# refresh-bio/colord

Hardware: AMD Instinct MI355X
Metric: input Gbases/s + archive size vs ref, ONT 50 Gb at 1/2/4/8 MI355X (higher is better)
Workload: dtype u64

## Files before the change

colord_amd/_native.py:

```python
from __future__ import annotations
import ctypes as C
import os

os.environ.setdefault("GPU_MAX_HW_QUEUES", "32")
_HERE = os.path.dirname(os.path.abspath(__file__))
LIB_PATH = os.environ.get("COLORD_HIP_LIBRARY") or os.path.join(_HERE, "libcolord_hip.so")

CL_OK, CL_E_INVALID, CL_E_HIP, CL_E_CAPACITY, CL_E_NOMEM, CL_E_UNSUPPORTED, CL_E_MISMATCH = 0, -1, -2, -3, -4, -5, -6


class ColordHipError(RuntimeError):
    def __init__(self, status, msg):
        super().__init__(f"colord_hip error {status}: {msg}")
        self.status = status


class QualParams(C.Structure):
    _fields_ = [("mode", C.c_int32), ("source", C.c_int32), ("level", C.c_int32), ("n_fwd", C.c_uint32), ("fwd", C.c_uint32 * 8),
                ("n_rev", C.c_uint32), ("rev", C.c_uint32 * 8)]


class KmerStats(C.Structure):
    _fields_ = [("n_reads", C.c_uint64), ("tot_kmers", C.c_uint64), ("n_unique", C.c_uint64),
                ("n_unique_counted", C.c_uint64), ("total_count_filtered", C.c_uint64)]


class Digest(C.Structure):
    _fields_ = [("reads", C.c_uint64), ("symbols", C.c_uint64), ("sum", C.c_uint64)]

    def triple(self):
        return self.reads, self.symbols, self.sum


class Report(C.Structure):
    _fields_ = [("reads", C.c_uint64), ("bases", C.c_uint64), ("base_count", C.c_uint64 * 5), ("len_min", C.c_uint64), ("len_max", C.c_uint64),
                ("len_hist", C.c_uint64 * 33), ("len_bases", C.c_uint64 * 33), ("has_qual", C.c_uint64), ("q_reads", C.c_uint64), ("q_symbols", C.c_uint64),
                ("mean_q_hist", C.c_uint64 * 96), ("q_joint", (C.c_uint64 * 96) * 96)]

    def as_dict(self):
        import numpy as np
        out = {}
        for name, t in self._fields_:
            v = getattr(self, name)
            out[name] = int(v) if t is C.c_uint64 else np.ctypeslib.as_array(v).copy()
        return out


_P = C.c_void_p
class CompressParams(C.Structure):
    _fields_ = [("k", C.c_uint32), ("f", C.c_uint32), ("ci", C.c_uint32), ("cs", C.c_uint32), ("c", C.c_uint32),
                ("anchor_len", C.c_uint32), ("min_part_alt", C.c_uint32), ("max_rec", C.c_uint32), ("min_anchors", C.c_uint32),
                ("level", C.c_int32), ("source", C.c_int32), ("sparse", C.c_int32),
                ("sparse_g", C.c_double), ("sparse_exponent", C.c_double),
                ("cost_mult", C.c_double), ("frac_always", C.c_double), ("frac_min", C.c_double), ("max_matches_mult", C.c_double)]


class CompressInfo(C.Structure):
    _fields_ = [(n, C.c_uint64) for n in ("n_reads", "n_bases", "tot_kmers", "n_kept_kmers", "n_refs", "n_anchors", "tuple_bytes", "dna_bytes", "qual_bytes")] + \
               [("sparse_range", C.c_uint32), ("pad", C.c_uint32)]


_EXCH_GATHER_HOST = C.CFUNCTYPE(C.c_int32, C.c_void_p, C.POINTER(C.c_uint64), C.c_uint32, C.POINTER(C.c_uint64))
_EXCH_A2AV = C.CFUNCTYPE(C.c_int32, C.c_void_p, C.c_void_p, C.POINTER(C.c_uint64), C.c_void_p, C.POINTER(C.c_uint64))
_EXCH_GATHERV = C.CFUNCTYPE(C.c_int32, C.c_void_p, C.c_void_p, C.c_uint64, C.c_void_p, C.POINTER(C.c_uint64))


class Exchange(C.Structure):
    _fields_ = [("user", C.c_void_p), ("rank", C.c_uint32), ("world", C.c_uint32),
                ("all_gather_host", _EXCH_GATHER_HOST), ("all_to_all_v", _EXCH_A2AV), ("all_gather_v", _EXCH_GATHERV)]


_SIG = {
    "cl_ctx_create": (C.c_int32, [C.c_int, C.POINTER(_P)]),
    "cl_ctx_destroy": (None, [_P]),
    "cl_last_error": (C.c_char_p, [_P]),
    "cl_ctx_stream": (_P, [_P]),
    "cl_ctx_last_kernel_ms": (C.c_int32, [_P, C.c_char_p, C.POINTER(C.c_double), C.POINTER(C.c_uint32)]),
    "cl_ctx_set_timing": (None, [_P, C.c_int]),
    "cl_ctx_set_verify": (None, [_P, C.c_int]),
    "cl_ctx_verified": (C.c_int32, [_P, C.POINTER(C.c_uint64), C.POINTER(C.c_uint64)]),
    "cl_ctx_gap_paths": (C.c_int32, [_P, C.POINTER(C.c_uint64), C.c_uint32]),
    "cl_ctx_set_verify_streams": (None, [_P, C.c_int]),
    "cl_ctx_verified_streams": (C.c_int32, [_P, C.POINTER(C.c_uint64), C.POINTER(C.c_uint64), C.POINTER(C.c_uint64)]),
    "cl_compressor_verified_streams": (C.c_int32, [_P, C.POINTER(C.c_uint64), C.POINTER(C.c_uint64), C.POINTER(C.c_uint64)]),
    "cl_ctx_set_digest": (None, [_P, C.c_int]),
    "cl_ctx_digest": (C.c_int32, [_P, C.POINTER(Digest), C.POINTER(Digest)]),
    "cl_compressor_digest": (C.c_int32, [_P, C.POINTER(Digest), C.POINTER(Digest)]),
    "cl_ctx_set_digest_values": (None, [_P, C.c_int]),
    "cl_ctx_digest_values": (C.c_int32, [_P, C.POINTER(Digest)]),
    "cl_compressor_digest_values": (C.c_int32, [_P, C.POINTER(Digest)]),
    "cl_digest_qual_values": (C.c_int32, [_P, C.POINTER(QualParams), _P, _P, _P, C.c_uint64, C.POINTER(Digest)]),
    "cl_qual_values": (C.c_int32, [_P, C.POINTER(QualParams), _P, _P, _P, _P, C.c_uint64]),
    "cl_qual_values_host": (C.c_int32, [C.POINTER(QualParams), _P, _P, C.c_uint64, _P]),
    "cl_digest_qual_values_host": (C.c_int32, [_P, _P, C.c_uint64, C.c_uint64, C.POINTER(Digest)]),
    "cl_report_clear": (None, [C.POINTER(Report)]),
    "cl_report_add": (None, [C.POINTER(Report), C.POINTER(Report)]),
    "cl_report_bases": (C.c_int32, [_P, _P, C.POINTER(Report)]),
    "cl_report_quals": (C.c_int32, [_P, C.POINTER(QualParams), _P, _P, _P, C.c_uint64, C.c_uint32, C.POINTER(Report)]),
    "cl_report_bases_host": (C.c_int32, [_P, _P, C.c_uint64, C.POINTER(Report)]),
    "cl_report_quals_host": (C.c_int32, [C.POINTER(QualParams), _P, _P, C.c_uint64, C.POINTER(Report)]),
    "cl_report_values_host": (C.c_int32, [_P, _P, C.c_uint64, C.POINTER(Report)]),
    "cl_ctx_set_report": (None, [_P, C.c_int]),
    "cl_ctx_report": (C.c_int32, [_P, C.POINTER(Report)]),
    "cl_compressor_report": (C.c_int32, [_P, C.POINTER(Report)]),
    "cl_digest_bases": (C.c_int32, [_P, _P, C.c_uint64, C.POINTER(Digest)]),
    "cl_digest_quals": (C.c_int32, [_P, C.POINTER(QualParams), _P, _P, _P, C.c_uint64, C.POINTER(Digest)]),
    "cl_digest_bases_host": (C.c_int32, [_P, _P, C.c_uint64, C.c_uint64, C.POINTER(Digest)]),
    "cl_digest_bytes_host": (C.c_int32, [C.c_uint32, _P, _P, C.c_uint64, C.c_uint64, C.POINTER(Digest)]),
    "cl_qual_decoder_set_digest": (C.c_int32, [_P, C.c_int, C.c_uint64]),
    "cl_qual_decoder_digest": (C.c_int32, [_P, C.POINTER(Digest)]),
    "cl_es_expand": (C.c_int32, [_P, _P, _P, _P, _P, C.c_uint32, _P, C.c_uint64, _P, C.POINTER(C.c_uint64)]),
    "cl_es_verify": (C.c_int32, [_P, _P, _P, _P, _P, _P, C.POINTER(C.c_uint64), C.POINTER(C.c_uint32)]),
    "cl_compressor_verified": (C.c_int32, [_P, C.POINTER(C.c_uint64), C.POINTER(C.c_uint64)]),
    "cl_ctx_kernel_times": (C.c_int32, [_P, C.c_char_p, C.c_uint64, C.POINTER(C.c_uint64)]),
    "cl_reads_pack": (C.c_int32, [_P, _P, _P, C.c_uint32, C.c_int, C.POINTER(_P)]),
    "cl_reads_free": (None, [_P]),
    "cl_reads_count": (C.c_uint32, [_P]),
    "cl_reads_total_bases": (C.c_uint64, [_P]),
    "cl_reads_total_words": (C.c_uint64, [_P]),
    "cl_reads_packed": (_P, [_P]),
    "cl_reads_invalid": (_P, [_P]),
    "cl_reads_word_offsets": (_P, [_P]),
    "cl_reads_lengths": (_P, [_P]),
    "cl_reads_has_n": (_P, [_P]),
    "cl_reads_compact": (C.c_int32, [_P, _P, C.c_uint32, _P, C.c_uint64, C.POINTER(C.c_uint64)]),
    "cl_kmer_scan": (C.c_int32, [_P, _P, C.c_uint32, C.c_uint32, _P, C.c_uint64, C.POINTER(C.c_uint64)]),
    "cl_kmer_count_filter": (C.c_int32, [_P, _P, C.c_uint64, C.c_uint32, C.c_uint32, C.c_uint32, C.POINTER(_P), C.POINTER(KmerStats)]),
    "cl_kmer_set_create": (C.c_int32, [_P, _P, _P, C.c_uint64, C.c_uint32, C.POINTER(_P)]),
    "cl_kmer_set_free": (None, [_P]),
    "cl_kmer_set_size": (C.c_uint64, [_P]),
    "cl_kmer_set_keys": (_P, [_P]),
    "cl_kmer_set_counts": (_P, [_P]),
    "cl_kmer_set_check": (C.c_int32, [_P, _P, _P, C.c_uint64, _P]),
    "cl_accepted_kmers": (C.c_int32, [_P, _P, _P, C.c_uint32, C.c_uint32, C.POINTER(_P)]),
    "cl_kmer_lists_free": (None, [_P]),
    "cl_kmer_lists_reads": (C.c_uint32, [_P]),
    "cl_kmer_lists_total": (C.c_uint64, [_P]),
    "cl_kmer_lists_offsets": (_P, [_P]),
    "cl_kmer_lists_kmers": (_P, [_P]),
    "cl_kmer_lists_ids": (_P, [_P]),
    "cl_kmer_lists_pos": (_P, [_P]),
    "cl_ref_accept": (C.c_int32, [C.c_uint32, C.c_uint32, C.c_uint32, C.c_double, _P]),
    "cl_index_build": (C.c_int32, [_P, _P, _P, _P, C.c_uint32, C.c_uint32, C.POINTER(_P)]),
    "cl_index_entries_of": (C.c_int32, [_P, _P, _P, C.c_uint32, _P, _P, C.c_uint64, C.POINTER(C.c_uint64), _P, C.POINTER(C.c_uint32)]),
    "cl_index_build_pairs": (C.c_int32, [_P, _P, _P, _P, C.c_uint64, _P, C.c_uint32, C.c_uint32, C.c_uint32, C.c_uint32, C.POINTER(_P)]),
    "cl_index_free": (None, [_P]),
    "cl_index_n_refs": (C.c_uint32, [_P]),
    "cl_index_entries": (C.c_uint64, [_P]),
    "cl_index_ref_rank": (_P, [_P]),
    "cl_candidates": (C.c_int32, [_P, _P, _P, C.c_uint32, _P, _P, _P]),
    "cl_candidates_common": (C.c_int32, [_P, _P, _P, C.c_uint32, _P, _P, _P, _P, C.c_uint64, C.POINTER(C.c_uint64)]),
    "cl_qual_coder_create": (C.c_int32, [_P, C.POINTER(QualParams), C.POINTER(_P)]),
    "cl_qual_coder_ctx": (_P, [_P]),
    "cl_qual_coder_free": (None, [_P]),
    "cl_qual_coder_set_domain_symbols": (C.c_int32, [_P, C.c_uint64]),
    "cl_qual_coder_domains": (C.c_int32, [_P, _P, C.c_uint64, C.POINTER(C.c_uint64)]),
    "cl_qual_coder_model": (C.c_int32, [_P, C.c_uint32, C.c_uint64, _P, C.c_uint32, C.POINTER(C.c_uint32)]),
    "cl_qual_coder_groups": (C.c_int32, [_P, C.POINTER(C.c_uint64)]),
    "cl_compressor_set_qual_domain_symbols": (C.c_int32, [_P, C.c_uint64]),
    "cl_compressor_qual_domains": (C.c_int32, [_P, _P, C.c_uint64, C.POINTER(C.c_uint64)]),
    "cl_qual_decode_domains": (C.c_int32, [_P, C.POINTER(QualParams), _P, _P, _P, C.c_uint64, _P, _P, C.c_uint32, _P, C.c_uint32, C.c_uint32, _P, _P, C.c_uint64, _P, C.c_uint64]),
    "cl_qual_encode": (C.c_int32, [_P, _P, _P, _P, _P, _P, _P, C.c_uint32, _P, C.c_uint64, _P, C.POINTER(C.c_uint64)]),
    "cl_anchor_candidates": (C.c_int32, [_P, _P, _P, _P, _P, C.c_uint32, C.c_uint32, C.c_double, C.c_double, C.c_double, C.c_uint32, C.POINTER(_P)]),
    "cl_anchor_candidates_hifi": (C.c_int32, [_P, _P, _P, _P, _P, C.c_uint32, C.c_uint32, C.c_double, C.c_double, C.c_double, C.c_uint32, C.c_uint32, C.c_uint32, _P, _P, C.POINTER(_P)]),
    "cl_anchors_free": (None, [_P]),
    "cl_anchors_total": (C.c_uint64, [_P]),
    "cl_anchors_n_cands": (_P, [_P]),
    "cl_anchors_cands": (_P, [_P]),
    "cl_anchors_cand_offsets": (_P, [_P]),
    "cl_anchors_data": (_P, [_P]),
    "cl_encode_plain": (C.c_int32, [_P, _P, _P, C.c_uint64, _P, _P, C.POINTER(C.c_uint64)]),
    "cl_reads_select": (C.c_int32, [_P, _P, _P, C.POINTER(_P)]),
    "cl_reads_from_arena": (C.c_int32, [_P, _P, _P, _P, C.c_uint32, C.POINTER(_P)]),
    "cl_estimator_logs": (C.c_int32, [_P, _P, _P, C.c_uint64, _P]),
    "cl_es_flags": (C.c_int32, [_P, _P, _P, _P, _P, _P]),
    "cl_id_coder_create": (C.c_int32, [C.c_int32, C.POINTER(_P)]),
    "cl_id_coder_free": (None, [_P]),
    "cl_id_coder_error": (C.c_char_p, [_P]),
    "cl_id_encode_part": (C.c_int32, [_P, _P, _P, _P, C.c_uint32, _P, C.c_uint64, C.POINTER(C.c_uint64)]),
    "cl_compress_shard": (C.c_int32, [_P, C.POINTER(CompressParams), _P, _P, _P, _P, C.c_uint32, _P, C.c_uint32, _P, _P, _P, C.c_uint64, _P, _P, C.c_uint64, _P,
                                      C.POINTER(CompressInfo)]),
    "cl_candidates_at": (C.c_int32, [_P, _P, _P, _P, C.c_uint32, _P, _P, _P]),
    "cl_compressor_create": (C.c_int32, [_P, _P, C.POINTER(CompressParams), C.POINTER(QualParams), C.POINTER(Exchange), C.c_uint64, C.POINTER(_P)]),
    "cl_compressor_free": (None, [_P]),
    "cl_compressor_count_add": (C.c_int32, [_P, _P]),
    "cl_compressor_count_finish": (C.c_int32, [_P, C.POINTER(KmerStats)]),
    "cl_compressor_refs_add": (C.c_int32, [_P, _P]),
    "cl_compressor_refs_finish": (C.c_int32, [_P]),
    "cl_compressor_encode": (C.c_int32, [_P, _P, _P, _P, _P, C.c_uint32, _P, C.c_uint32, _P, C.c_uint64, _P, _P, C.c_uint64, _P, C.POINTER(CompressInfo)]),
    "cl_compressor_genome_add": (C.c_int32, [_P, _P]),
    "cl_compressor_pseudo_reads": (C.c_int32, [_P, _P]),
    "cl_genome_encode": (C.c_int32, [_P, _P, C.c_uint32, _P, C.c_uint64, C.POINTER(C.c_uint64)]),
    "cl_genome_decode": (C.c_int32, [_P, C.c_uint64, C.c_uint32, _P, C.c_uint64, _P, C.POINTER(C.c_uint64)]),
    "cl_genome_md5": (C.c_int32, [_P, _P, C.c_uint32, _P]),
    "cl_compressor_prepare": (C.c_int32, [_P, _P, _P, C.c_uint32]),
    "cl_compressor_prepare_parts": (C.c_int32, [_P, _P, _P, C.c_uint32, _P, C.c_uint32, _P, _P]),
    "cl_compressor_info": (C.c_int32, [_P, C.POINTER(KmerStats), C.POINTER(C.c_uint64), C.POINTER(C.c_uint64), C.POINTER(C.c_uint64), C.POINTER(C.c_uint32), C.POINTER(C.c_uint32)]),
    "cl_dna_decoder_create": (C.c_int32, [C.c_uint32, C.c_int32, C.c_uint32, C.c_uint32, C.c_int32, C.c_uint32, C.c_double, C.POINTER(_P)]),
    "cl_dna_decoder_free": (None, [_P]),
    "cl_dna_decoder_error": (C.c_char_p, [_P]),
    "cl_dna_decoder_add_ref": (C.c_int32, [_P, _P, C.c_uint32]),
    "cl_dna_decoder_new_domain": (C.c_int32, [_P]),
    "cl_dna_decode_part": (C.c_int32, [_P, _P, C.c_uint64, C.c_uint32, _P, C.c_uint64, _P, C.POINTER(C.c_uint64)]),
    "cl_qual_decoder_create": (C.c_int32, [C.POINTER(QualParams), C.POINTER(_P)]),
    "cl_qual_decoder_free": (None, [_P]),
    "cl_qual_decoder_new_domain": (C.c_int32, [_P]),
    "cl_qual_decode_part": (C.c_int32, [_P, _P, C.c_uint64, _P, _P, C.c_uint32, _P]),
    "cl_id_decoder_create": (C.c_int32, [C.c_int32, C.POINTER(_P)]),
    "cl_id_decoder_free": (None, [_P]),
    "cl_id_decode_part": (C.c_int32, [_P, _P, C.c_uint64, C.c_uint32, _P, C.c_uint64, _P, _P, C.POINTER(C.c_uint64)]),
    "cl_encode_reads": (C.c_int32, [_P, _P, _P, _P, C.c_uint32, C.c_uint32, C.c_uint32, C.c_uint32, C.c_double, _P, C.c_uint32, _P, C.c_uint64, _P, _P, C.POINTER(C.c_uint64)]),
    "cl_dna_coder_create": (C.c_int32, [_P, C.c_uint32, C.c_int32, C.c_uint32, C.POINTER(_P)]),
    "cl_dna_coder_free": (None, [_P]),
    "cl_dna_coder_model": (C.c_int32, [_P, C.c_uint32, C.c_uint64, _P]),
    "cl_dna_encode": (C.c_int32, [_P, _P, _P, _P, _P, _P, C.c_uint32, _P, C.c_uint32, _P, C.c_uint64, _P, C.POINTER(C.c_uint64)]),
    "cl_sort_u64": (C.c_int32, [_P, _P, C.c_uint64, C.c_uint32, C.c_uint32]),
    "cl_sort_u64_u32": (C.c_int32, [_P, _P, _P, C.c_uint64, C.c_uint32, C.c_uint32]),
    "cl_sort_u32": (C.c_int32, [_P, _P, C.c_uint64, C.c_uint32, C.c_uint32]),
    "cl_sort_u32_u32": (C.c_int32, [_P, _P, _P, C.c_uint64, C.c_uint32, C.c_uint32]),
    "cl_sort_swap_u32_u32": (C.c_int32, [_P, _P, _P, C.c_uint64, C.c_uint32, C.c_uint32, _P, _P]),
    "cl_sort_swap_u64_u32": (C.c_int32, [_P, _P, _P, C.c_uint64, C.c_uint32, C.c_uint32, _P, _P]),
    "cl_scan_u32": (C.c_int32, [_P, _P, C.c_uint64, C.POINTER(C.c_uint64)]),
    "cl_scan_u32_u64": (C.c_int32, [_P, _P, _P, C.c_uint64, C.POINTER(C.c_uint64)]),
    "cl_run_starts_u32": (C.c_int32, [_P, _P, C.c_uint64, C.c_uint32, _P, C.c_uint64, C.POINTER(C.c_uint64)]),
    "cl_run_starts_u64": (C.c_int32, [_P, _P, C.c_uint64, C.c_uint32, _P, C.c_uint64, C.POINTER(C.c_uint64)]),
}

_lib = None


def load():
    global _lib
    if _lib is None:
        if not os.path.exists(LIB_PATH):
            raise ColordHipError(CL_E_HIP, f"{LIB_PATH} is missing: run `make -C colord_amd/csrc` "
                                 "(or __graft_entry__.build()); there is no CPU fallback")
        lib = C.CDLL(LIB_PATH)
        for name, (res, args) in _SIG.items():
            fn = getattr(lib, name)
            fn.restype, fn.argtypes = res, args
        _lib = lib
    return _lib


def exported_names():
    return sorted(_SIG)
```

colord_amd/csrc/anchors.hip:

```cpp
#include "common.hpp"
#include "objects.hpp"
#include <algorithm>

struct cl_anchors {
	cl_ctx* ctx = nullptr;
	uint32_t n_reads = 0, c = 0;
	uint64_t n_anchors = 0;
	DevBuf<uint32_t> n_cands;
	DevBuf<uint32_t> cand;
	DevBuf<uint64_t> cand_off;
	DevBuf<uint32_t> anchors;
};

namespace {

struct Arena { const uint64_t* packed; const uint64_t* word_off; const uint32_t* lens; };

__device__ inline uint64_t mmer_at(const Arena& A, uint64_t wb, uint32_t p, uint32_t m)
{
	const uint64_t* w = A.packed + wb + (p >> 5);
	const uint32_t j = p & 31;
	const uint64_t hi = w[0], lo = w[1];
	const uint32_t s = 128 - 2 * (j + m);
	const uint64_t v = (s >= 64) ? (hi >> (s - 64)) : ((hi << (64 - s)) | (lo >> s));
// ... 686 lines not shown
		if (ku != 2) { sel_task[n] = (trc + ku) | 0x80000000u; sel_tot[n] = k_tot[trc + ku]; sel_n[n] = k_n[trc + ku]; ++n; continue; }
		int pick = -1;
		if (arc && afw) pick = t_tot[tfw] > t_tot[trc] ? 1 : 0;
		else if (arc) pick = 0;
		else if (afw) pick = 1;
		if (pick >= 0) { sel_task[n] = trc + (uint32_t)pick; sel_tot[n] = t_tot[trc + pick]; sel_n[n] = t_nanch[trc + pick]; ++n; }
	}
	for (uint32_t i = 1; i < n; ++i)
	{
		uint32_t xt = sel_task[i], xv = sel_tot[i], xn = sel_n[i]; uint32_t j = i;
		while (j > 0 && xv > sel_tot[j - 1]) { sel_task[j] = sel_task[j - 1]; sel_tot[j] = sel_tot[j - 1]; sel_n[j] = sel_n[j - 1]; --j; }
		sel_task[j] = xt; sel_tot[j] = xv; sel_n[j] = xn;
	}
	o_ncand[r] = n;
	for (uint32_t i = 0; i < c; ++i)
	{
		const uint64_t s = (uint64_t)r * c + i;
		if (i < n)
		{
			const uint32_t t = sel_task[i] & 0x7fffffffu, slot = (t / 2) % c;
			o_cand[4 * s] = cand_refs[(uint64_t)r * c + slot]; o_cand[4 * s + 1] = (t & 1) == 0 ? 1u : 0u;
			o_cand[4 * s + 2] = sel_tot[i]; o_cand[4 * s + 3] = sel_n[i];
			o_task[(uint64_t)rl * c + i] = sel_task[i]; o_count[(uint64_t)rl * c + i] = sel_n[i];
		}
		else { o_cand[4 * s] = ~0u; o_cand[4 * s + 1] = 0; o_cand[4 * s + 2] = 0; o_cand[4 * s + 3] = 0; o_task[(uint64_t)rl * c + i] = ~0u; o_count[(uint64_t)rl * c + i] = 0; }
	}
}
__global__ void k_copy_fix(const uint32_t* __restrict__ o_task, const uint64_t* __restrict__ slot_off, uint64_t n_slots,
                           const uint64_t* __restrict__ pair_off, const uint32_t* __restrict__ anch, uint64_t dst_base, uint32_t* __restrict__ out,
                           TaskCfg cfg, const uint32_t* __restrict__ kanch, const uint64_t* __restrict__ common_off, uint64_t common_base)
{
	const uint64_t s = (uint64_t)blockIdx.x * blockDim.x + threadIdx.x;
	if (s >= n_slots) return;
	const uint32_t tm = o_task[s];
	if (tm == ~0u) return;
	const uint32_t t = tm & 0x7fffffffu;
	const uint32_t n = (uint32_t)(slot_off[s + 1] - slot_off[s]);
	const uint32_t* src = anch + 3 * pair_off[t];
	if (tm & 0x80000000u)
	{
		const uint64_t gs = (uint64_t)cfg.r0 * cfg.c + t / 2;
		const uint64_t o = common_off[gs] - common_base; const uint32_t nk = (uint32_t)(common_off[gs + 1] - common_off[gs]);
		src = kanch + 6 * o + (uint64_t)(t & 1) * 3 * nk;
	}
	uint32_t* dst = out + 3 * (dst_base + slot_off[s]);
	for (uint32_t i = 0; i < 3 * n; ++i) dst[i] = src[i];
	for (uint32_t i = 0; i + 1 < n; ++i)
	{
		const uint32_t end = dst[3 * i + 2] + dst[3 * i];
		if (dst[3 * (i + 1) + 2] < end) { const uint32_t d = end - dst[3 * (i + 1) + 2]; dst[3 * (i + 1) + 2] += d; dst[3 * (i + 1)] -= d; dst[3 * (i + 1) + 1] += d; }
	}
	for (uint32_t i = 0; i + 1 < n; ++i)
	{
		const uint32_t end = dst[3 * i + 1] + dst[3 * i];
		if (dst[3 * (i + 1) + 1] < end) { const uint32_t d = end - dst[3 * (i + 1) + 1]; dst[3 * (i + 1) + 1] += d; dst[3 * (i + 1)] -= d; dst[3 * (i + 1) + 2] += d; }
	}
}
__global__ void k_add_u64(uint64_t* v, uint64_t n, uint64_t c) { uint64_t i = (uint64_t)blockIdx.x * blockDim.x + threadIdx.x; if (i < n) v[i] += c; }
}

extern "C" cl_status cl_anchor_candidates_hifi(cl_ctx* ctx, const cl_reads* reads, const cl_reads* refs, const uint32_t* d_cand_refs, const uint32_t* d_cand_n,
                                               uint32_t c, uint32_t anchor_len, double frac_always, double frac_min, double max_matches_mult,
                                               uint32_t min_anchors, uint32_t kmer_len, uint32_t modulo, const uint64_t* d_common_off, const uint64_t* d_common, cl_anchors** out);
extern "C" cl_status cl_anchor_candidates(cl_ctx* ctx, const cl_reads* reads, const cl_reads* refs, const uint32_t* d_cand_refs, const uint32_t* d_cand_n,
                                          uint32_t c, uint32_t anchor_len, double frac_always, double frac_min, double max_matches_mult,
                                          uint32_t min_anchors, cl_anchors** out)
{
	return cl_anchor_candidates_hifi(ctx, reads, refs, d_cand_refs, d_cand_n, c, anchor_len, frac_always, frac_min, max_matches_mult, min_anchors, 0, 0, nullptr, nullptr, out);
}
extern "C" cl_status cl_anchor_candidates_hifi(cl_ctx* ctx, const cl_reads* reads, const cl_reads* refs, const uint32_t* d_cand_refs, const uint32_t* d_cand_n,
                                               uint32_t c, uint32_t anchor_len, double frac_always, double frac_min, double max_matches_mult,
                                               uint32_t min_anchors, uint32_t kmer_len, uint32_t modulo, const uint64_t* d_common_off, const uint64_t* d_common, cl_anchors** out)
{
	if (!ctx || !reads || !refs || !d_cand_refs || !d_cand_n || !out) return cl_fail(ctx, CL_E_INVALID, "cl_anchor_candidates: null argument");
	const bool hifi = d_common_off != nullptr;
	if (hifi && (kmer_len < 2 || kmer_len > 28 || modulo == 0)) return cl_fail(ctx, CL_E_INVALID, "cl_anchor_candidates_hifi: 2 <= kmer_len <= 28, modulo >= 1");
	if (c == 0 || c > 16 || anchor_len < 2 || anchor_len > 28) return cl_fail(ctx, CL_E_INVALID, "cl_anchor_candidates: 1 <= c <= 16, 2 <= anchor_len <= 28");
	HIP_TRY(ctx, hipSetDevice(ctx->device));
	const uint32_t nr = reads->n_reads, m = anchor_len;
	cl_anchors* X = new cl_anchors(); X->ctx = ctx; X->n_reads = nr; X->c = c;
	std::unique_ptr<cl_anchors> guard(X);
	DEV_ALLOC(ctx, X->n_cands, nr); DEV_ALLOC(ctx, X->cand, (uint64_t)nr * c * 4); DEV_ALLOC(ctx, X->cand_off, (uint64_t)nr * c + 1);
	Arena A{ reads->packed.p, reads->word_off.p, reads->lens.p }, R{ refs->packed.p, refs->word_off.p, refs->lens.p };
	std::vector<uint32_t> h_len(nr);
	if (nr) HIP_TRY(ctx, hipMemcpy(h_len.data(), reads->lens.p, (uint64_t)nr * 4, hipMemcpyDeviceToHost));
	auto bits_for = [](uint64_t v) -> uint32_t { uint32_t b = 1; while ((1ull << b) <= v) ++b; return b; };
	uint32_t max_ref_len = 0;
	if (refs->n_reads)
	{
		std::vector<uint32_t> rl(refs->n_reads);
		HIP_TRY(ctx, hipMemcpy(rl.data(), refs->lens.p, (uint64_t)refs->n_reads * 4, hipMemcpyDeviceToHost));
		for (uint32_t l : rl) max_ref_len = std::max(max_ref_len, l);
	}
	const uint32_t pr_bits = bits_for(max_ref_len);
	const uint64_t BATCH_BASES = 1ull << 28;
	std::vector<DevBuf<uint32_t>> chunks; std::vector<uint64_t> chunk_n;
	uint64_t total_anchors = 0;
	double pairs_per_base = 0.5;
	struct TableBatch {
		uint32_t r0 = 0, r1 = 0, pe = 1; uint64_t acc = 0, nsum = 0;
		DevBuf<uint32_t> n_distinct, next, err; DevBuf<uint64_t> toff, noff; DevBuf<EncSlot> slots; DevBuf<uint2> bins;
		std::vector<uint2> h_work; DevBuf<uint2> work;
		struct SideSync { hipStream_t s = nullptr; ~SideSync() { if (s) (void)hipStreamSynchronize(s); } } sync;
	};
	HIP_TRY(ctx, cl_side_stream(ctx, ctx->side));
	constexpr uint32_t LDS_N_A = 12288, LDS_N_B = 24576, LDS_NT = 1024;
	uint32_t lds_max_n = 0;
	if (const char* e = getenv("COLORD_HIP_ANCHORS_LDS")) lds_max_n = atoi(e) <= 0 ? 0u : (uint32_t)atoi(e) <= LDS_N_A ? LDS_N_A : LDS_N_B;
	const uint32_t match_seg = getenv("COLORD_HIP_MATCH_SEG") ? (uint32_t)std::max(0, atoi(getenv("COLORD_HIP_MATCH_SEG"))) : 16384u;
	const uint32_t lds_dbg = getenv("COLORD_HIP_LDS_DBG") ? (uint32_t)atoi(getenv("COLORD_HIP_LDS_DBG")) : 0u;
	auto prepare = [&](uint32_t r0, std::unique_ptr<TableBatch>& out) -> cl_status {
		out = std::make_unique<TableBatch>();
		TableBatch& B = *out;
		uint32_t r1 = r0; uint64_t acc = 0;
		uint32_t mx = 0;
		while (r1 < nr && (r1 == r0 || acc + h_len[r1] <= BATCH_BASES))
		{
			const uint32_t pe = bits_for(std::max(mx, h_len[r1]));
			if (r1 > r0 && pe + pr_bits + bits_for((r1 - r0 + 1) * 2 * c) > 64) break;
			mx = std::max(mx, h_len[r1]); acc += h_len[r1]; ++r1;
		}
		B.r0 = r0; B.r1 = r1; B.acc = acc; B.pe = bits_for(mx);
		for (uint32_t r = r0; r < r1; ++r)
			for (uint32_t sg = 0, ns = match_segments(h_len[r] >= m ? h_len[r] - m + 1 : 0, match_seg); sg < ns; ++sg) B.h_work.push_back(make_uint2(r - r0, sg));
		if (B.pe + pr_bits + bits_for((r1 - r0) * 2 * c) > 64) return cl_fail(ctx, CL_E_UNSUPPORTED, "cl_anchor_candidates: a read and its candidates are too long for 64-bit match keys");
		const uint32_t nb = r1 - r0;
		const uint32_t table_x4 = 8;
		LaunchOn on(ctx, ctx->side);
		B.sync.s = ctx->side;
		DevBuf<uint32_t> tsize, nsize, err; DEV_ALLOC(ctx, tsize, nb); DEV_ALLOC(ctx, nsize, nb); DEV_ALLOC(ctx, err, 1); DEV_ALLOC(ctx, B.n_distinct, nb);
		HIP_TRY(ctx, hipMemsetAsync(err.p, 0, 4, ctx->side));
		LAUNCH(ctx, k_table_sizes, grid_for(nb, 256), 256, (const uint32_t*)reads->lens.p, (const uint8_t*)reads->has_n.p, d_cand_n, r0, r1, m, table_x4, lds_max_n, tsize.p, nsize.p, err.p);
		DEV_ALLOC(ctx, B.toff, (uint64_t)nb + 1); DEV_ALLOC(ctx, B.noff, (uint64_t)nb + 1);
		uint64_t tsum = 0;
		CL_TRY(dev_exclusive_scan_u64(ctx, tsize.p, B.toff.p, nb, &tsum));
		CL_TRY(dev_exclusive_scan_u64(ctx, nsize.p, B.noff.p, nb, &B.nsum));
		uint32_t herr = 0; HIP_TRY(ctx, hipMemcpyAsync(&herr, err.p, 4, hipMemcpyDeviceToHost, ctx->side)); HIP_TRY(ctx, hipStreamSynchronize(ctx->side));
		DEV_ALLOC(ctx, B.slots, tsum); DEV_ALLOC(ctx, B.next, B.nsum); DEV_ALLOC(ctx, B.bins, B.nsum); DEV_ALLOC(ctx, B.err, 1);
		DEV_ALLOC(ctx, B.work, B.h_work.size() + 1);
		if (!B.h_work.empty()) HIP_TRY(ctx, hipMemcpyAsync(B.work.p, B.h_work.data(), B.h_work.size() * sizeof(uint2), hipMemcpyHostToDevice, ctx->side));
		HIP_TRY(ctx, hipMemsetAsync(B.n_distinct.p, 0, (uint64_t)nb * 4, ctx->side));
		HIP_TRY(ctx, hipMemsetAsync(B.err.p, 0, 4, ctx->side));
		EncTable T{ B.slots.p, B.toff.p, B.next.p, B.noff.p };
		LAUNCHB(ctx, B.nsum * (0.25 + 16.0) , k_table_insert, nb, INS_T, A, r0, r1, m, T, B.n_distinct.p, B.bins.p, B.err.p);
		HIP_TRY(ctx, hipGetLastError());
		return CL_OK;
	};
	std::unique_ptr<TableBatch> cur, nxt;
	if (nr) CL_TRY(prepare(0, cur));
	while (cur)
	{
		const uint32_t r0 = cur->r0, r1 = cur->r1; const uint64_t acc = cur->acc;
		const uint32_t nb = r1 - r0, n_tasks = nb * 2 * c;
		TaskCfg cfg{ r0, r1, c, m, cur->pe, pr_bits, frac_always, frac_min, max_matches_mult };
		HIP_TRY(ctx, hipStreamSynchronize(ctx->stream));
		HIP_TRY(ctx, hipStreamSynchronize(ctx->side));
		cur->sync.s = nullptr;
		{ uint32_t herr = 0; HIP_TRY(ctx, hipMemcpy(&herr, cur->err.p, 4, hipMemcpyDeviceToHost)); if (herr) return cl_fail(ctx, CL_E_UNSUPPORTED, "cl_anchor_candidates: a region of an m-mer table overflowed"); }
		DevBuf<uint32_t>& n_distinct = cur->n_distinct;
		EncTable T{ cur->slots.p, cur->toff.p, cur->next.p, cur->noff.p };
		DevBuf<uint32_t> pair_cnt; DEV_ALLOC(ctx, pair_cnt, (uint64_t)n_tasks + 1);
		DevBuf<uint64_t> pair_off; DEV_ALLOC(ctx, pair_off, (uint64_t)n_tasks + 1);
		DevBuf<unsigned long long> d_np; DEV_ALLOC(ctx, d_np, 4);
		DevBuf<uint64_t> pairs;
		uint64_t n_pairs = 0;
		for (uint64_t cap = (uint64_t)(pairs_per_base * 1.25 * (double)acc) + (1u << 20);;)
		{
			DEV_ALLOC(ctx, pairs, cap);
			HIP_TRY(ctx, hipMemsetAsync(d_np.p, 0, 32, ctx->stream));
			if (lds_max_n)
			{
				LAUNCH_NAMED(ctx, "k_match_lds<12288>", (k_match_lds<LDS_N_A, 2048, LDS_NT, 8>), nb, LDS_NT, A, R, cfg, 0u, (const uint8_t*)reads->has_n.p, d_cand_refs, d_cand_n, n_distinct.p, nb, d_np.p, cap, pairs.p, lds_dbg);
				if (lds_max_n > LDS_N_A)
					LAUNCH_NAMED(ctx, "k_match_lds<24576>", (k_match_lds<LDS_N_B, 4096, LDS_NT, 4>), nb, LDS_NT, A, R, cfg, LDS_N_A, (const uint8_t*)reads->has_n.p, d_cand_refs, d_cand_n, n_distinct.p, nb, d_np.p, cap, pairs.p, lds_dbg);
			}
			LAUNCHB(ctx, 0.0, k_match, (uint32_t)cur->h_work.size(), 256, A, R, T, cfg, d_cand_refs, d_cand_n, (const uint32_t*)n_distinct.p, (const uint2*)cur->work.p, (uint32_t)cur->h_work.size(), match_seg, d_np.p, cap, pairs.p);
			HIP_TRY(ctx, hipGetLastError());
			unsigned long long h_np2[2] = { 0, 0 };
			HIP_TRY(ctx, hipMemcpyAsync(h_np2, d_np.p, 16, hipMemcpyDeviceToHost, ctx->stream));
			if (r1 < nr && !nxt) CL_TRY(prepare(r1, nxt));
			HIP_TRY(ctx, hipStreamSynchronize(ctx->stream));
			const unsigned long long h_np = h_np2[0];
			n_pairs = h_np;
			if (ctx->timing && !ctx->pending_bytes.empty()) ctx->pending_bytes.back() = (double)h_np2[1] * 8.25 + (double)std::min<uint64_t>(h_np, cap) * 8.0;
			if (getenv("COLORD_HIP_ANCHOR_DEBUG")) fprintf(stderr, "[anchors] batch reads %u..%u bases %llu: pairs %llu cap %llu\n", r0, r1, (unsigned long long)acc, h_np, (unsigned long long)cap);
			if (n_pairs >= (1ull << 32)) return cl_fail(ctx, CL_E_UNSUPPORTED, "cl_anchor_candidates: batch produces >= 2^32 match pairs");
			if (n_pairs <= cap) break;
			cap = n_pairs;
		}
		if (acc) pairs_per_base = std::max(pairs_per_base, (double)n_pairs / (double)acc);
		DevBuf<int> tf, ts, pred; DEV_ALLOC(ctx, tf, n_pairs); DEV_ALLOC(ctx, ts, n_pairs); DEV_ALLOC(ctx, pred, n_pairs);
		DevBuf<uint32_t> anch; DEV_ALLOC(ctx, anch, 3 * n_pairs);
		DevBuf<uint32_t> t_nanch, t_tot; DEV_ALLOC(ctx, t_nanch, n_tasks); DEV_ALLOC(ctx, t_tot, n_tasks);
		if (n_pairs)
		{
			uint32_t tb = 1; while ((1ull << tb) < n_tasks) ++tb;
			CL_TRY(dev_sort_pairs(ctx, pairs.p, nullptr, n_pairs, 0, cfg.pe + cfg.pr + tb));
		}
		LAUNCH(ctx, k_task_pairs, grid_for((uint64_t)n_tasks + 1, 256), 256, (const uint64_t*)pairs.p, n_pairs, A, cfg, (const uint32_t*)n_distinct.p, n_tasks, pair_off.p, pair_cnt.p);
		LAUNCHB(ctx, n_pairs * 32.0, k_lis_anchors, grid_for(n_tasks, 64), 64, A, R, cfg, d_cand_refs, n_tasks, (const uint64_t*)pair_off.p, (const uint32_t*)pair_cnt.p, (const uint64_t*)pairs.p,
			tf.p, ts.p, pred.p, anch.p, t_nanch.p, t_tot.p, (uint32_t)(getenv("COLORD_HIP_LIS_DBG") ? atoi(getenv("COLORD_HIP_LIS_DBG")) : 0));
		HIP_TRY(ctx, hipGetLastError());
		const uint64_t n_slots = (uint64_t)nb * c;
		DevBuf<uint64_t> k_sorted; DevBuf<uint32_t> k_tab, kanch, k_n, k_tot; DevBuf<uint8_t> k_use;
		uint64_t common_base = 0;
		if (hifi)
		{
			uint64_t hb[2] = { 0, 0 };
			HIP_TRY(ctx, hipMemcpy(&hb[0], d_common_off + (uint64_t)r0 * c, 8, hipMemcpyDeviceToHost));
			HIP_TRY(ctx, hipMemcpy(&hb[1], d_common_off + (uint64_t)r1 * c, 8, hipMemcpyDeviceToHost));
			common_base = hb[0];
			const uint64_t nk = hb[1] - hb[0];
			DEV_ALLOC(ctx, k_sorted, nk + 1); DEV_ALLOC(ctx, k_tab, 8 * nk + 8); DEV_ALLOC(ctx, kanch, 6 * nk + 6);
			DEV_ALLOC(ctx, k_n, 2 * n_slots); DEV_ALLOC(ctx, k_tot, 2 * n_slots); DEV_ALLOC(ctx, k_use, n_slots);
			KmerArgs ka{ d_common, d_common_off, k_sorted.p, k_tab.p, kanch.p, k_n.p, k_tot.p, k_use.p, common_base, kmer_len, make_modtest(modulo) };
			LAUNCH(ctx, k_kmer_anchors, grid_for(n_slots, 64), 64, A, R, cfg, d_cand_refs, d_cand_n, (const uint8_t*)reads->has_n.p, (const uint32_t*)n_distinct.p, ka);
			HIP_TRY(ctx, hipGetLastError());
		}
		DevBuf<uint32_t> o_task, o_count; DEV_ALLOC(ctx, o_task, n_slots); DEV_ALLOC(ctx, o_count, n_slots);
		LAUNCH(ctx, k_select, grid_for(nb, 128), 128, cfg, d_cand_refs, d_cand_n, min_anchors, (const uint32_t*)t_nanch.p, (const uint32_t*)t_tot.p,
			(const uint8_t*)(hifi ? k_use.p : nullptr), (const uint32_t*)k_n.p, (const uint32_t*)k_tot.p,
			X->n_cands.p, X->cand.p, o_task.p, o_count.p);
		DevBuf<uint64_t> slot_off; DEV_ALLOC(ctx, slot_off, n_slots + 1);
		uint64_t n_here = 0;
		CL_TRY(dev_exclusive_scan_u64(ctx, o_count.p, slot_off.p, n_slots, &n_here));
		DevBuf<uint32_t> chunk; DEV_ALLOC(ctx, chunk, 3 * n_here);
		LAUNCH(ctx, k_copy_fix, grid_for(n_slots, 128), 128, (const uint32_t*)o_task.p, (const uint64_t*)slot_off.p, n_slots, (const uint64_t*)pair_off.p,
			(const uint32_t*)anch.p, (uint64_t)0, chunk.p, cfg, (const uint32_t*)kanch.p, d_common_off, common_base);
		HIP_TRY(ctx, hipMemcpyAsync(X->cand_off.p + (uint64_t)r0 * c, slot_off.p, n_slots * 8, hipMemcpyDeviceToDevice, ctx->stream));
		if (total_anchors) LAUNCH(ctx, k_add_u64, grid_for(n_slots, 256), 256, X->cand_off.p + (uint64_t)r0 * c, n_slots, total_anchors);
		HIP_TRY(ctx, hipGetLastError());
		HIP_TRY(ctx, hipStreamSynchronize(ctx->stream));
		chunks.push_back(std::move(chunk)); chunk_n.push_back(n_here);
		total_anchors += n_here;
		cur = std::move(nxt);
	}
	X->n_anchors = total_anchors;
	DEV_ALLOC(ctx, X->anchors, 3 * total_anchors);
	uint64_t o = 0;
	for (size_t i = 0; i < chunks.size(); ++i)
	{
		if (chunk_n[i]) HIP_TRY(ctx, hipMemcpyAsync(X->anchors.p + 3 * o, chunks[i].p, chunk_n[i] * 12, hipMemcpyDeviceToDevice, ctx->stream));
		o += chunk_n[i];
	}
	HIP_TRY(ctx, hipMemcpyAsync(X->cand_off.p + (uint64_t)nr * c, &total_anchors, 8, hipMemcpyHostToDevice, ctx->stream));
	HIP_TRY(ctx, hipStreamSynchronize(ctx->stream));
	cl_timing_collect(ctx);
	*out = guard.release();
	return CL_OK;
}
extern "C" void cl_anchors_free(cl_anchors* a) { delete a; }
extern "C" uint64_t cl_anchors_total(const cl_anchors* a) { return a->n_anchors; }
extern "C" const uint32_t* cl_anchors_n_cands(const cl_anchors* a) { return a->n_cands.p; }
extern "C" const uint32_t* cl_anchors_cands(const cl_anchors* a) { return a->cand.p; }
extern "C" const uint64_t* cl_anchors_cand_offsets(const cl_anchors* a) { return a->cand_off.p; }
extern "C" const uint32_t* cl_anchors_data(const cl_anchors* a) { return a->anchors.p; }
```

colord_amd/csrc/capi.hip:

```cpp
#include "common.hpp"
#include "objects.hpp"
#include <cmath>
#include <random>

extern "C" cl_status cl_ctx_create(int device, cl_ctx** out)
{
	if (!out) return CL_E_INVALID;
	*out = nullptr;
	int n = 0;
	hipError_t e = hipGetDeviceCount(&n);
	if (e != hipSuccess || n <= 0) { fprintf(stderr, "colord_hip: no HIP device available (%s)\n", hipGetErrorString(e)); return CL_E_HIP; }
	if (device < 0 || device >= n) return CL_E_INVALID;
	if (hipSetDevice(device) != hipSuccess) return CL_E_HIP;
	cl_ctx* c = new cl_ctx(device);
	if (hipStreamCreateWithFlags(&c->stream, hipStreamNonBlocking) != hipSuccess) { cl_ctx_destroy(c); return CL_E_HIP; }
	hipDeviceProp_t p;
	if (hipGetDeviceProperties(&p, device) == hipSuccess) c->n_cu = p.multiProcessorCount;
	*out = c;
	return CL_OK;
}
void cl_ctx_set_priority(cl_ctx* c, int level, int role)
{
	if (!c) return;
	(void)hipSetDevice(c->device);
// ... 24 lines not shown
			if (cl_stream_create(c, &ns) != hipSuccess) { (void)hipGetLastError(); (void)hipStreamCreateWithFlags(&ns, hipStreamNonBlocking); }
			s->store(ns);
		}
}
namespace { __global__ void k_poison_check(const uint32_t* __restrict__ p, uint64_t n, unsigned long long* __restrict__ bad)
{
	uint64_t mine = 0;
	for (uint64_t i = (uint64_t)blockIdx.x * blockDim.x + threadIdx.x; i < n; i += (uint64_t)gridDim.x * blockDim.x) mine += p[i] != 0xCDCDCDCDu;
	if (mine) atomicAdd(bad, (unsigned long long)mine);
} }
void cl_ctx_poison(cl_ctx* c, void* p, uint64_t bytes)
{
	if (!c || !c->stream) return;
	(void)hipSetDevice(c->device);
	if (hipMemsetAsync(p, 0xCD, bytes, c->stream) != hipSuccess) { (void)hipGetLastError(); return; }
	(void)hipStreamSynchronize(c->stream);
}
uint64_t cl_pool_poison_check(void* p, uint64_t bytes)
{
	static unsigned long long* d_bad = nullptr;
	if (!d_bad && hipMalloc((void**)&d_bad, 8) != hipSuccess) { (void)hipGetLastError(); return 0; }
	(void)hipDeviceSynchronize();
	(void)hipMemset(d_bad, 0, 8);
	hipLaunchKernelGGL(k_poison_check, dim3(1024), dim3(256), 0, nullptr, (const uint32_t*)p, bytes / 4, d_bad);
	unsigned long long h = 0;
	if (hipGetLastError() != hipSuccess || hipMemcpy(&h, d_bad, 8, hipMemcpyDeviceToHost) != hipSuccess) { (void)hipGetLastError(); fprintf(stderr, "colord_hip: pool poison: the check itself failed\n"); return 0; }
	return h;
}
void cl_ctx_drain(cl_ctx* c)
{
	if (!c) return;
	(void)hipSetDevice(c->device);
	for (hipStream_t s : { c->stream, c->side.load(std::memory_order_acquire), c->side2.load(std::memory_order_acquire), c->side3.load(std::memory_order_acquire) }) if (s) (void)hipStreamSynchronize(s);
}
int cl_ctx_fence(cl_ctx* c, hipEvent_t* ev)
{
	if (!c) return 0;
	int n = 0;
	for (hipStream_t s : { c->stream, c->side.load(std::memory_order_acquire), c->side2.load(std::memory_order_acquire), c->side3.load(std::memory_order_acquire) }) if (s && n < 4) { if (hipEventRecord(ev[n], s) == hipSuccess) ++n; else (void)hipGetLastError(); }
	return n;
}
extern "C" void cl_ctx_destroy(cl_ctx* c)
{
	if (!c) return;
	for (cl_ctx* l : c->lanes) cl_ctx_destroy(l);
	c->lanes.clear();
	if (c->prep) { cl_ctx_destroy(c->prep); c->prep = nullptr; }
	if (c->qprep) { cl_ctx_destroy(c->qprep); c->qprep = nullptr; }
	(void)hipSetDevice(c->device);
	cl_ctx_drain(c);
	for (auto& kv : c->scan_ctl) if (kv.second.p) c->pool.put(kv.second.p, kv.second.got, c->pool_id);
	c->scan_ctl.clear();
	c->pool.drop_owner(c->pool_id);
	for (auto& p : c->pending) { (void)hipEventDestroy(p.second.first); (void)hipEventDestroy(p.second.second); }
	for (auto e : c->ev_pool) (void)hipEventDestroy(e);
	if (c->stream) (void)hipStreamDestroy(c->stream);
	for (std::atomic<hipStream_t>* s : { &c->side, &c->side2, &c->side3 }) if (hipStream_t x = s->load()) (void)hipStreamDestroy(x);
	if (c->inv_tab) (void)hipFree(c->inv_tab);
	if (c->slots_h) (void)hipHostFree(c->slots_h);
	delete c->report_acc;
	const int dev = c->device;
	delete c;
	cl_device_pool_release(dev);
}
extern "C" const char* cl_last_error(const cl_ctx* c) { return c ? c->err.c_str() : "null context"; }
extern "C" void* cl_ctx_stream(cl_ctx* c) { return c ? (void*)c->stream : nullptr; }
extern "C" void cl_ctx_set_timing(cl_ctx* c, int on) { if (c) c->timing = on != 0; }
extern "C" void cl_ctx_set_verify(cl_ctx* c, int on) { if (c) c->verify = on != 0; }
extern "C" cl_status cl_ctx_verified(const cl_ctx* c, uint64_t* reads, uint64_t* bases)
{
	if (!c) return CL_E_INVALID;
	uint64_t r = c->verified_reads.load(), b = c->verified_bases.load();
	for (const cl_ctx* l : c->lanes) { r += l->verified_reads.load(); b += l->verified_bases.load(); }
	if (reads) *reads = r;
	if (bases) *bases = b;
	return CL_OK;
}
extern "C" cl_status cl_ctx_gap_paths(const cl_ctx* c, uint64_t* out, uint32_t cap)
{
	if (!c || (!out && cap)) return CL_E_INVALID;
	for (uint32_t i = 0; i < cap && i < 11; ++i) out[i] = c->gap_paths[i];
	return CL_OK;
}
extern "C" cl_status cl_dna_coder_model(const cl_dna_coder* d, uint32_t family, uint64_t context, uint32_t* out)
{
	if (!d || !out) return CL_E_INVALID;
	return cl_dna_model_read(d, family, context, out);
}
extern "C" cl_status cl_qual_coder_model(const cl_qual_coder* q, uint32_t family, uint64_t context, uint32_t* out, uint32_t cap, uint32_t* n_out)
{
	if (!q || !out || !n_out) return CL_E_INVALID;
	return cl_qual_model_read(q, family, context, out, cap, n_out);
}
extern "C" void cl_ctx_set_verify_streams(cl_ctx* c, int on) { if (c) c->verify_streams = on != 0; }
extern "C" cl_status cl_ctx_verified_streams(const cl_ctx* c, uint64_t* parts, uint64_t* symbols, uint64_t* bytes)
{
	if (!c) return CL_E_INVALID;
	if (parts) *parts = c->verified_stream_parts.load();
	if (symbols) *symbols = c->verified_stream_symbols.load();
	if (bytes) *bytes = c->verified_stream_bytes.load();
	return CL_OK;
}
extern "C" cl_status cl_ctx_last_kernel_ms(const cl_ctx* c, const char* kernel, double* ms, uint32_t* launches)
{
	if (!c || !kernel) return CL_E_INVALID;
	auto it = c->times.find(kernel);
	if (it == c->times.end()) { if (ms) *ms = 0; if (launches) *launches = 0; return CL_E_INVALID; }
	if (ms) *ms = it->second.ms;
	if (launches) *launches = it->second.launches;
	return CL_OK;
}

extern "C" cl_status cl_ctx_kernel_times(cl_ctx* c, char* buf, uint64_t cap, uint64_t* needed)
{
	if (!c) return CL_E_INVALID;
	cl_timing_collect(c);
	std::string out;
	for (auto& kv : c->times) out += kv.first + "\t" + std::to_string(kv.second.ms) + "\t" + std::to_string(kv.second.launches) + "\t" + std::to_string(kv.second.bytes) + "\t" + std::to_string(kv.second.cells) + "\n";
	if (needed) *needed = out.size() + 1;
	if (!buf || cap < out.size() + 1) return CL_E_CAPACITY;
	memcpy(buf, out.c_str(), out.size() + 1);
	c->times.clear();
	return CL_OK;
}

extern "C" cl_status cl_ref_accept(uint32_t n_reads, uint32_t n_pseudo, uint32_t range, double exponent, uint8_t* h_out)
{
	if (!h_out || range == 0) return CL_E_INVALID;
	std::mt19937 mt;
	std::uniform_real_distribution<double> dist(0.0, 1.0);
	for (uint64_t i = 0; i < (uint64_t)n_reads + n_pseudo; ++i)
	{
		if (i < n_pseudo) { h_out[i] = 1; continue; }
		uint32_t range_no = (uint32_t)((i - n_pseudo) / range);
		double p = std::pow(1.0 / (range_no + 1ul), exponent);
		h_out[i] = dist(mt) <= p;
	}
	return CL_OK;
}

extern "C" cl_status cl_sort_u64(cl_ctx* ctx, uint64_t* d_keys, uint64_t n, uint32_t begin_bit, uint32_t end_bit)
{
	if (!ctx || (!d_keys && n)) return cl_fail(ctx, CL_E_INVALID, "cl_sort_u64: null argument");
	HIP_TRY(ctx, hipSetDevice(ctx->device));
	cl_timing_begin(ctx);
	cl_status s = dev_sort_pairs(ctx, d_keys, nullptr, n, begin_bit, end_bit);
	cl_timing_collect(ctx);
	return s;
}
extern "C" cl_status cl_sort_u64_u32(cl_ctx* ctx, uint64_t* d_keys, uint32_t* d_vals, uint64_t n, uint32_t begin_bit, uint32_t end_bit)
{
	if (!ctx || ((!d_keys || !d_vals) && n)) return cl_fail(ctx, CL_E_INVALID, "cl_sort_u64_u32: null argument");
	HIP_TRY(ctx, hipSetDevice(ctx->device));
	cl_timing_begin(ctx);
	cl_status s = dev_sort_pairs(ctx, d_keys, d_vals, n, begin_bit, end_bit);
	cl_timing_collect(ctx);
	return s;
}

extern "C" cl_status cl_scan_u32(cl_ctx* ctx, uint32_t* d_data, uint64_t n, uint64_t* h_total)
{
	if (!ctx || (!d_data && n)) return cl_fail(ctx, CL_E_INVALID, "cl_scan_u32: null argument");
	HIP_TRY(ctx, hipSetDevice(ctx->device));
	cl_timing_begin(ctx);
	cl_status s = dev_exclusive_scan_u32(ctx, d_data, n, h_total);
	hipError_t e = hipStreamSynchronize(ctx->stream);
	cl_timing_collect(ctx);
	if (s == CL_OK) HIP_TRY(ctx, e);
	return s;
}
extern "C" cl_status cl_scan_u32_u64(cl_ctx* ctx, const uint32_t* d_in, uint64_t* d_out, uint64_t n, uint64_t* h_total)
{
	if (!ctx || !d_out || (!d_in && n)) return cl_fail(ctx, CL_E_INVALID, "cl_scan_u32_u64: null argument");
	HIP_TRY(ctx, hipSetDevice(ctx->device));
	cl_timing_begin(ctx);
	cl_status s = dev_exclusive_scan_u64(ctx, d_in, d_out, n, h_total);
	hipError_t e = hipStreamSynchronize(ctx->stream);
	cl_timing_collect(ctx);
	if (s == CL_OK) HIP_TRY(ctx, e);
	return s;
}
extern "C" cl_status cl_run_starts_u32(cl_ctx* ctx, const uint32_t* d_keys, uint64_t n, uint32_t shift, uint32_t* d_seg, uint64_t seg_cap, uint64_t* h_n_runs)
{
	if (!ctx || !h_n_runs || ((!d_keys || !d_seg) && n)) return cl_fail(ctx, CL_E_INVALID, "cl_run_starts_u32: null argument");
	HIP_TRY(ctx, hipSetDevice(ctx->device));
	cl_timing_begin(ctx);
	cl_status s = dev_run_starts_u32(ctx, d_keys, n, shift, d_seg, seg_cap, h_n_runs);
	cl_timing_collect(ctx);
	return s;
}
extern "C" cl_status cl_run_starts_u64(cl_ctx* ctx, const uint64_t* d_keys, uint64_t n, uint32_t shift, uint32_t* d_seg, uint64_t seg_cap, uint64_t* h_n_runs)
{
	if (!ctx || !h_n_runs || ((!d_keys || !d_seg) && n)) return cl_fail(ctx, CL_E_INVALID, "cl_run_starts_u64: null argument");
	HIP_TRY(ctx, hipSetDevice(ctx->device));
	cl_timing_begin(ctx);
	cl_status s = dev_run_starts_u64(ctx, d_keys, n, shift, d_seg, seg_cap, h_n_runs);
	cl_timing_collect(ctx);
	return s;
}
extern "C" cl_status cl_sort_u32(cl_ctx* ctx, uint32_t* d_keys, uint64_t n, uint32_t begin_bit, uint32_t end_bit)
{
	return cl_sort_u32_u32(ctx, d_keys, nullptr, n, begin_bit, end_bit);
}
extern "C" cl_status cl_sort_u32_u32(cl_ctx* ctx, uint32_t* d_keys, uint32_t* d_vals, uint64_t n, uint32_t begin_bit, uint32_t end_bit)
{
	if (!ctx || (!d_keys && n)) return cl_fail(ctx, CL_E_INVALID, "cl_sort_u32_u32: null argument");
	HIP_TRY(ctx, hipSetDevice(ctx->device));
	cl_timing_begin(ctx);
	cl_status s = dev_sort_keys32_pairs(ctx, d_keys, d_vals, n, begin_bit, end_bit);
	cl_timing_collect(ctx);
	return s;
}
namespace {
template<typename K, typename Sort>
cl_status sort_swap_copy(cl_ctx* ctx, const char* who, const K* d_keys_in, const uint32_t* d_vals_in, uint64_t n, uint32_t begin_bit, uint32_t end_bit, K* d_keys_out, uint32_t* d_vals_out, Sort sort)
{
	if (!ctx || ((!d_keys_in || !d_vals_in || !d_keys_out || !d_vals_out) && n)) return cl_fail(ctx, CL_E_INVALID, std::string(who) + ": null argument");
	HIP_TRY(ctx, hipSetDevice(ctx->device));
	cl_timing_begin(ctx);
	DevBuf<K> keys; DEV_ALLOC(ctx, keys, n);
	DevBuf<uint32_t> vals; DEV_ALLOC(ctx, vals, n);
	if (n)
	{
		HIP_TRY(ctx, hipMemcpyAsync(keys.p, d_keys_in, n * sizeof(K), hipMemcpyDeviceToDevice, ctx->stream));
		HIP_TRY(ctx, hipMemcpyAsync(vals.p, d_vals_in, n * 4, hipMemcpyDeviceToDevice, ctx->stream));
	}
	cl_status s = sort(ctx, keys, vals, n, begin_bit, end_bit);
	if (s == CL_OK && n)
	{
		HIP_TRY(ctx, hipMemcpyAsync(d_keys_out, keys.p, n * sizeof(K), hipMemcpyDeviceToDevice, ctx->stream));
		HIP_TRY(ctx, hipMemcpyAsync(d_vals_out, vals.p, n * 4, hipMemcpyDeviceToDevice, ctx->stream));
	}
	hipError_t e = hipStreamSynchronize(ctx->stream);
	cl_timing_collect(ctx);
	if (s == CL_OK) HIP_TRY(ctx, e);
	return s;
}
}
extern "C" cl_status cl_sort_swap_u32_u32(cl_ctx* ctx, const uint32_t* d_keys_in, const uint32_t* d_vals_in, uint64_t n, uint32_t begin_bit, uint32_t end_bit, uint32_t* d_keys_out, uint32_t* d_vals_out)
{
	return sort_swap_copy<uint32_t>(ctx, "cl_sort_swap_u32_u32", d_keys_in, d_vals_in, n, begin_bit, end_bit, d_keys_out, d_vals_out, dev_sort_keys32_pairs_swap);
}
extern "C" cl_status cl_sort_swap_u64_u32(cl_ctx* ctx, const uint64_t* d_keys_in, const uint32_t* d_vals_in, uint64_t n, uint32_t begin_bit, uint32_t end_bit, uint64_t* d_keys_out, uint32_t* d_vals_out)
{
	return sort_swap_copy<uint64_t>(ctx, "cl_sort_swap_u64_u32", d_keys_in, d_vals_in, n, begin_bit, end_bit, d_keys_out, d_vals_out, dev_sort_pairs_swap);
}
```

colord_amd/csrc/common.hpp:

```cpp
#pragma once
#ifdef CL_HOST_DEBUG
#define CL_DEV __host__ __device__
#else
#define CL_DEV __device__
#endif
#include <hip/hip_runtime.h>
#include <cstdint>
#include <cstdio>
#include <cstring>
#include <string>
#include <vector>
#include <algorithm>
#include <map>
#include <deque>
#include <mutex>
#include <atomic>
#include <condition_variable>
#include <thread>
#include <chrono>
#include "../../include/colord_hip.h"

#define CL_WAVE 64

struct KernelTime { double ms = 0; uint32_t launches = 0; double bytes = 0, cells = 0; };

struct cl_ctx;
void cl_ctx_drain(cl_ctx* c);
void cl_ctx_set_priority(cl_ctx* c, int level, int role = -1);
int cl_ctx_fence(cl_ctx* c, hipEvent_t* ev);
void cl_ctx_poison(cl_ctx* c, void* p, uint64_t bytes);
uint64_t cl_pool_poison_check(void* p, uint64_t bytes);
static inline bool cl_pool_poison() { static const bool on = getenv("COLORD_HIP_POOL_POISON") != nullptr; return on; }
struct DevPool {
	struct Ext { uint64_t len; int32_t owner; uint64_t clock; bool poisoned = false; };
	struct Slab { char* base = nullptr; uint64_t size = 0, free_bytes = 0; std::map<uint64_t, Ext> ext; };
	std::mutex mu;
	std::vector<Slab> slabs;
	std::vector<cl_ctx*> owners; std::vector<uint64_t> drained; uint64_t clock = 0;
	std::vector<uint32_t> pinned; std::condition_variable pin_cv;
	struct Fence { uint64_t clock; hipEvent_t ev[4]; int n; };
	std::vector<std::deque<Fence>> fences; std::vector<uint32_t> since_fence; std::vector<hipEvent_t> spare_events;
	uint64_t reserved = 0, live_bytes = 0, peak_live = 0, peak_total = 0; uint32_t n_mallocs = 0, n_drains = 0;
	uint64_t n_poison_checks = 0, n_poison_bad = 0;
	static constexpr uint64_t ALIGN = 256, PAD = 256, SLAB_MIN = 256ull << 20, SLAB_MAX = 4ull << 30;
	int32_t add_owner(cl_ctx* c) { std::lock_guard<std::mutex> l(mu); owners.push_back(c); drained.push_back(0); fences.emplace_back(); since_fence.push_back(0); pinned.push_back(0); return (int32_t)owners.size() - 1; }
	void drop_owner(int32_t id)
	{
		std::unique_lock<std::mutex> l(mu);
		if (id < 0 || (size_t)id >= owners.size()) return;
		pin_cv.wait(l, [&] { return pinned[id] == 0; });
		owners[id] = nullptr; drained[id] = ~0ull;
		for (auto& f : fences[id]) for (int i = 0; i < f.n; ++i) spare_events.push_back(f.ev[i]);
		fences[id].clear();
	}
	void poll_fences_locked(int32_t id)
	{
		auto& q = fences[id];
		while (!q.empty())
		{
			bool done = true;
			for (int i = 0; i < q.front().n && done; ++i) done = hipEventQuery(q.front().ev[i]) == hipSuccess;
			if (!done) { (void)hipGetLastError(); break; }
			if (drained[id] < q.front().clock) drained[id] = q.front().clock;
			for (int i = 0; i < q.front().n; ++i) spare_events.push_back(q.front().ev[i]);
			q.pop_front();
		}
	}
	bool clean(const Ext& e) const { return e.owner < 0 || e.clock <= drained[e.owner]; }
	bool usable(const Ext& e, int32_t who) const { return e.owner == who || clean(e); }
	uint64_t shed_locked(uint64_t want)
	{
		uint64_t freed = 0;
		while (freed < want)
		{
			size_t best = slabs.size();
			for (size_t i = 0; i < slabs.size(); ++i) if (slabs[i].free_bytes == slabs[i].size && (best == slabs.size() || slabs[i].size > slabs[best].size)) best = i;
			if (best == slabs.size()) break;
			(void)hipFree(slabs[best].base); freed += slabs[best].size; reserved -= slabs[best].size;
			slabs.erase(slabs.begin() + best);
		}
		return freed;
	}
	void make_room(uint64_t r, bool dbg)
	{
		size_t fr = 0, tot = 0;
		if (hipMemGetInfo(&fr, &tot) != hipSuccess) { (void)hipGetLastError(); return; }
		const uint64_t need = r + (1ull << 30);
		if (fr >= need) return;
		const uint64_t freed = shed_locked(need - fr);
		if (dbg) fprintf(stderr, "[pool] device has %.1f GB free, %.3f GB wanted: gave back %.3f GB of free slabs\n", fr / 1e9, r / 1e9, freed / 1e9);
	}
	void coalesce_locked()
	{
		for (Slab& S : slabs)
			for (auto it = S.ext.begin(); it != S.ext.end();)
			{
				auto nx = std::next(it);
				if (nx == S.ext.end()) break;
				if (it->first + it->second.len == nx->first && (it->second.owner == nx->second.owner || (clean(it->second) && clean(nx->second))))
				{
					if (it->second.owner != nx->second.owner) { it->second.owner = -1; it->second.clock = 0; } else it->second.clock = std::max(it->second.clock, nx->second.clock);
					it->second.poisoned = it->second.poisoned && nx->second.poisoned;
// ... 106 lines not shown
					{
						const uint64_t upto = clock;
						drain_unlocked(lock, fo);
						if (drained[fo] < upto) drained[fo] = upto;
					}
				}
				if (!got_it) return e;
				if (dbg) fprintf(stderr, "[pool] no slab of %.3f GB to be had: waited for a block of %.3f GB\n", sz / 1e9, r / 1e9);
				live_bytes += r; if (live_bytes > peak_live) peak_live = live_bytes;
				return hipSuccess;
			}
			Slab S; S.base = (char*)base; S.size = sz; S.free_bytes = sz; S.ext.emplace(0, Ext{ sz, -1, 0 });
			slabs.push_back(std::move(S));
			reserved += sz; if (reserved > peak_total) peak_total = reserved;
			if (!carve(r, who, out, nullptr)) return hipErrorOutOfMemory;
		}
		live_bytes += r; if (live_bytes > peak_live) peak_live = live_bytes;
		return hipSuccess;
	}
	void put(void* p, uint64_t r, int32_t who)
	{
		std::lock_guard<std::mutex> lock(mu);
		for (Slab& S : slabs)
		{
			if ((char*)p < S.base || (char*)p >= S.base + S.size) continue;
			uint64_t off = (uint64_t)((char*)p - S.base);
			Ext me{ r, who, ++clock };
			if (cl_pool_poison() && who >= 0 && owners[who]) { cl_ctx_poison(owners[who], p, r); me.poisoned = true; }
			auto nx = S.ext.lower_bound(off);
			if (nx != S.ext.begin()) { auto pv = std::prev(nx); if (pv->first + pv->second.len == off && pv->second.owner == who) { off = pv->first; me.len += pv->second.len; me.poisoned = me.poisoned && pv->second.poisoned; S.ext.erase(pv); } }
			if (nx != S.ext.end() && off + me.len == nx->first && nx->second.owner == who) { me.len += nx->second.len; me.poisoned = me.poisoned && nx->second.poisoned; S.ext.erase(nx); }
			S.ext.emplace(off, me);
			S.free_bytes += r; live_bytes -= r;
			if (who >= 0 && owners[who] && (++since_fence[who] >= 8 || r >= (64ull << 20)))
			{
				since_fence[who] = 0;
				poll_fences_locked(who);
				if (fences[who].size() < 64)
				{
					Fence f; f.clock = clock; f.n = 0;
					int have = 0;
					for (; have < 4; ++have) { if (spare_events.empty()) { hipEvent_t e; if (hipEventCreateWithFlags(&e, hipEventDisableTiming) != hipSuccess) { (void)hipGetLastError(); break; } spare_events.push_back(e); } f.ev[have] = spare_events.back(); spare_events.pop_back(); }
					if (have == 4) f.n = cl_ctx_fence(owners[who], f.ev);
					for (int i = f.n; i < have; ++i) spare_events.push_back(f.ev[i]);
					if (f.n > 0) fences[who].push_back(f);
				}
			}
			return;
		}
		if (reserved) fprintf(stderr, "colord_hip: pool released a block it does not own\n");
	}
	void trim()
	{
		std::lock_guard<std::mutex> lock(mu);
		if (cl_pool_poison()) fprintf(stderr, "[pool poison] %llu blocks checked at their hand-over to another context, %llu had lost the pattern\n", (unsigned long long)n_poison_checks, (unsigned long long)n_poison_bad);
		if (getenv("COLORD_HIP_POOL_DEBUG")) fprintf(stderr, "[pool] at trim: peak live %.1f GB, peak reserved %.1f GB, reserved %.1f GB in %zu slabs, %u hipMalloc calls, %u waits for another context's streams, still live %.3f GB\n", peak_live / 1e9, peak_total / 1e9, reserved / 1e9, slabs.size(), n_mallocs, n_drains, live_bytes / 1e9);
		for (auto& S : slabs) (void)hipFree(S.base);
		slabs.clear(); reserved = 0;
	}
};

static inline bool cl_pool_debug() { static const bool dbg = getenv("COLORD_HIP_POOL_DEBUG") != nullptr; return dbg; }

struct DevicePools { std::mutex mu; std::map<int, std::pair<DevPool*, int>> by_dev; };
inline DevicePools& cl_device_pools() { static DevicePools* p = new DevicePools; return *p; }
inline DevPool& cl_device_pool_acquire(int device)
{
	DevicePools& D = cl_device_pools();
	std::lock_guard<std::mutex> l(D.mu);
	auto& e = D.by_dev[device];
	if (!e.first) e.first = new DevPool();
	++e.second;
	return *e.first;
}
inline void cl_device_pool_release(int device)
{
	DevicePools& D = cl_device_pools();
	std::lock_guard<std::mutex> l(D.mu);
	auto it = D.by_dev.find(device);
	if (it == D.by_dev.end()) return;
	if (--it->second.second == 0) it->second.first->trim();
}

struct cl_ctx {
	DevPool& pool;
	int device = 0;
	int32_t pool_id = -1;
	explicit cl_ctx(int dev) : pool(cl_device_pool_acquire(dev)), device(dev) { pool_id = pool.add_owner(this); }
	hipStream_t stream = nullptr;
	hipStream_t launch = nullptr;
	int prio = 0;
	bool masked = false;
	int role = 0;
	std::atomic<hipStream_t> side{ nullptr };
	std::atomic<hipStream_t> side2{ nullptr };
	std::atomic<hipStream_t> side3{ nullptr };
	std::string err;
	bool timing = false;
	bool verify = false;
	std::atomic<uint64_t> verified_reads{ 0 }, verified_bases{ 0 };
	bool verify_streams = false;
	std::atomic<uint64_t> verified_stream_parts{ 0 }, verified_stream_symbols{ 0 }, verified_stream_bytes{ 0 };
	bool digest = false;
	cl_digest digest_dna{ 0, 0, 0 }, digest_qual{ 0, 0, 0 };
	bool digest_values = false;
	cl_digest digest_qval{ 0, 0, 0 };
	bool report = false;
	cl_report* report_acc = nullptr;
	uint64_t gap_paths[11] = { 0 };
	std::map<std::string, KernelTime> times;
	std::vector<std::pair<std::string, std::pair<hipEvent_t, hipEvent_t>>> pending;
	std::vector<double> pending_bytes, pending_cells;
	double next_bytes = 0, next_cells = 0;
	std::vector<hipEvent_t> ev_pool;
	int n_cu = 256;
	uint64_t* inv_tab = nullptr;
	uint64_t* slots_h = nullptr; uint64_t* slots_d = nullptr; uint32_t slot_next = 0;
	struct ScanCtl { unsigned long long* p = nullptr; uint64_t words = 0, got = 0; uint32_t gen = 0; unsigned long long tickets = 0; };
	std::map<void*, ScanCtl> scan_ctl;
	std::vector<cl_ctx*> lanes;
	cl_ctx* prep = nullptr;
	cl_ctx* qprep = nullptr;
};

static inline cl_status cl_fail(cl_ctx* c, cl_status s, const std::string& msg)
{
	if (c) c->err = msg;
	return s;
}

#define HIP_TRY(ctx, expr) do { hipError_t _e = (expr); if (_e != hipSuccess) { \
	return cl_fail((ctx), CL_E_HIP, std::string(#expr) + ": " + hipGetErrorString(_e) + " @" + __FILE__ + ":" + std::to_string(__LINE__)); } } while (0)
#define CL_TRY(expr) do { cl_status _s = (expr); if (_s != CL_OK) return _s; } while (0)

template<typename T> struct DevBuf {
	T* p = nullptr; uint64_t n = 0; uint64_t bytes = 0; DevPool* pool = nullptr; int32_t owner = -1;
	DevBuf() = default;
	DevBuf(const DevBuf&) = delete; DevBuf& operator=(const DevBuf&) = delete;
	DevBuf(DevBuf&& o) noexcept : p(o.p), n(o.n), bytes(o.bytes), pool(o.pool), owner(o.owner) { o.p = nullptr; o.n = 0; }
	DevBuf& operator=(DevBuf&& o) noexcept { if (this != &o) { release(); p = o.p; n = o.n; bytes = o.bytes; pool = o.pool; owner = o.owner; o.p = nullptr; o.n = 0; } return *this; }
	~DevBuf() { release(); }
	void release() { if (p) { if (pool) pool->put(p, bytes, owner); else (void)hipFree(p); } p = nullptr; n = 0; }
	hipError_t alloc(cl_ctx* c, uint64_t count);
};
template<typename T> hipError_t DevBuf<T>::alloc(cl_ctx* c, uint64_t count)
{
	release(); n = count; if (!count) count = 1;
	pool = &c->pool; owner = c->pool_id;
	void* q = nullptr;
	hipError_t e = pool->get(count * sizeof(T), &q, &bytes, owner);
	p = (T*)q;
	if (e != hipSuccess) { p = nullptr; n = 0; }
	return e;
}

#define DEV_ALLOC(ctx, buf, count) do { hipError_t _e = (buf).alloc((ctx), count); \
	if ((buf).bytes >= (1ull << 30) && cl_pool_debug()) fprintf(stderr, "[pool] %s:%d %s %.2f GB (live %.1f GB)\n", &__FILE__[sizeof(__FILE__) > 24 ? sizeof(__FILE__) - 24 : 0], __LINE__, #buf, (buf).bytes / 1e9, (ctx)->pool.live_bytes / 1e9); \
	if (_e != hipSuccess) \
	return cl_fail((ctx), CL_E_NOMEM, std::string("hipMalloc(" #buf ") of ") + std::to_string((uint64_t)(count)) + " elems: " + hipGetErrorString(_e)); } while (0)

static inline hipError_t cl_slot(cl_ctx* c, uint32_t n_words, uint64_t** h, uint64_t** d)
{
	constexpr uint32_t RING = 4096;
	if (!c->slots_h)
	{
		void* p = nullptr; void* dp = nullptr;
		hipError_t e = hipHostMalloc(&p, RING * 8, hipHostMallocMapped);
		if (e != hipSuccess) return e;
		e = hipHostGetDevicePointer(&dp, p, 0);
		if (e != hipSuccess) { (void)hipHostFree(p); return e; }
		memset(p, 0, RING * 8);
		c->slots_h = (uint64_t*)p; c->slots_d = (uint64_t*)dp;
	}
	if (n_words > RING) return hipErrorInvalidValue;
	if (c->slot_next + n_words > RING) c->slot_next = 0;
	*h = c->slots_h + c->slot_next; *d = c->slots_d + c->slot_next;
	c->slot_next += n_words;
	return hipSuccess;
}

static inline hipStream_t cl_launch_stream(const cl_ctx* c) { return c->launch ? c->launch : c->stream; }
struct LaunchOn { cl_ctx* c; hipStream_t prev; LaunchOn(cl_ctx* c_, hipStream_t s) : c(c_), prev(c_->launch) { c->launch = s; } ~LaunchOn() { c->launch = prev; } };
static inline bool cl_sync_debug() { static const bool d = getenv("COLORD_HIP_SYNC_DEBUG") != nullptr; return d; }
struct KernelTimer {
	cl_ctx* c; const char* name; hipEvent_t a = nullptr, b = nullptr;
	KernelTimer(cl_ctx* c_, const char* n) : c(c_), name(n)
	{
		if (!c->timing) return;
		auto get = [&]() { hipEvent_t e; if (!c->ev_pool.empty()) { e = c->ev_pool.back(); c->ev_pool.pop_back(); } else (void)hipEventCreate(&e); return e; };
		a = get(); b = get();
		(void)hipEventRecord(a, cl_launch_stream(c));
// ... 89 lines not shown
static inline void cl_timing_collect(cl_ctx* c, bool wait = false)
{
	if (!c->timing) return;
	size_t keep = 0;
	for (size_t i = 0; i < c->pending.size(); ++i)
	{
		auto& p = c->pending[i];
		bool done = true;
		if (wait) (void)hipEventSynchronize(p.second.second);
		else if (hipEventQuery(p.second.second) != hipSuccess) { (void)hipGetLastError(); done = false; }
		if (!done)
		{
			if (keep != i) { c->pending[keep] = std::move(p); c->pending_bytes[keep] = c->pending_bytes[i]; c->pending_cells[keep] = c->pending_cells[i]; }
			++keep;
			continue;
		}
		float ms = 0; (void)hipEventElapsedTime(&ms, p.second.first, p.second.second);
		std::string nm = p.first;
		if (!nm.empty() && nm.front() == '(' && nm.back() == ')') nm = nm.substr(1, nm.size() - 2);
		auto& t = c->times[nm]; t.ms += ms; t.launches += 1; t.bytes += c->pending_bytes[i]; t.cells += c->pending_cells[i];
		c->ev_pool.push_back(p.second.first); c->ev_pool.push_back(p.second.second);
	}
	c->pending.resize(keep); c->pending_bytes.resize(keep); c->pending_cells.resize(keep);
}

__host__ __device__ static inline uint64_t hash_mm(uint64_t x)
{
	x ^= x >> 33; x *= 0xff51afd7ed558ccdULL;
	x ^= x >> 33; x *= 0xc4ceb9fe1a85ec53ULL;
	x ^= x >> 33;
	return x;
}

struct ModTest { uint64_t low_mask, dinv, lim; uint32_t s; };
static inline ModTest make_modtest(uint32_t f)
{
	ModTest m; uint32_t s = 0; uint64_t d = f;
	while ((d & 1) == 0) { d >>= 1; ++s; }
	uint64_t inv = d;
	for (int i = 0; i < 6; ++i) inv *= 2 - d * inv;
	m.s = s; m.low_mask = (s ? ((1ULL << s) - 1) : 0); m.dinv = inv; m.lim = ~0ULL / d;
	return m;
}
__device__ static inline bool mod_is_zero(uint64_t h, const ModTest& m)
{
	return ((h & m.low_mask) == 0) && (((h >> m.s) * m.dinv) <= m.lim);
}

__device__ static inline uint32_t lane_id() { return threadIdx.x & 63; }
__device__ static inline uint64_t lanemask_lt() { return (1ULL << lane_id()) - 1; }

__device__ static inline uint32_t wave_incl_scan(uint32_t v)
{
#pragma unroll
	for (int d = 1; d < 64; d <<= 1) { uint32_t t = __shfl_up(v, d, 64); if ((int)lane_id() >= d) v += t; }
	return v;
}
__device__ static inline uint32_t wave_sum(uint32_t v)
{
#pragma unroll
	for (int d = 32; d > 0; d >>= 1) v += __shfl_xor(v, d, 64);
	return v;
}

__device__ static inline uint32_t block_excl_scan_256(uint32_t v, uint32_t* sh, uint32_t* total)
{
	uint32_t incl = wave_incl_scan(v);
	uint32_t w = threadIdx.x >> 6;
	__syncthreads();
	if (lane_id() == 63) sh[w] = incl;
	__syncthreads();
	uint32_t base = 0, tot = 0;
#pragma unroll
	for (uint32_t i = 0; i < 4; ++i) { uint32_t s = sh[i]; if (i < w) base += s; tot += s; }
	*total = tot;
	return base + incl - v;
}

cl_status dev_exclusive_scan_u32(cl_ctx* ctx, uint32_t* d_data, uint64_t n, uint64_t* h_total);
cl_status dev_exclusive_scan_u64(cl_ctx* ctx, const uint32_t* d_in, uint64_t* d_out, uint64_t n, uint64_t* h_total);
cl_status dev_run_starts_u32(cl_ctx* ctx, const uint32_t* d_keys, uint64_t n, uint32_t shift, uint32_t* d_seg, uint64_t seg_cap, uint64_t* h_n_runs);
cl_status dev_run_starts_u64(cl_ctx* ctx, const uint64_t* d_keys, uint64_t n, uint32_t shift, uint32_t* d_seg, uint64_t seg_cap, uint64_t* h_n_runs);
cl_status dev_sort_pairs(cl_ctx* ctx, uint64_t* d_keys, uint32_t* d_vals, uint64_t n, uint32_t begin_bit, uint32_t end_bit);
cl_status dev_sort_pairs_swap(cl_ctx* ctx, DevBuf<uint64_t>& keys, DevBuf<uint32_t>& vals, uint64_t n, uint32_t begin_bit, uint32_t end_bit);
cl_status dev_sort_keys32_pairs(cl_ctx* ctx, uint32_t* d_keys, uint32_t* d_vals, uint64_t n, uint32_t begin_bit, uint32_t end_bit);
cl_status dev_sort_keys32_pairs_swap(cl_ctx* ctx, DevBuf<uint32_t>& keys, DevBuf<uint32_t>& vals, uint64_t n, uint32_t begin_bit, uint32_t end_bit);

static inline uint32_t grid_for(uint64_t n, uint32_t per_block) { return (uint32_t)((n + per_block - 1) / per_block); }
```

colord_amd/csrc/kmer.hip:

```cpp
#include "common.hpp"
#include "objects.hpp"
static inline double cap_hint(uint64_t bases, uint32_t f) { return (double)bases / (f ? f : 1); }
#include <algorithm>

namespace {

__global__ void k_read_geometry(const uint64_t* __restrict__ off, uint32_t n_reads, uint32_t* __restrict__ lens,
                                uint32_t* __restrict__ words, uint32_t* __restrict__ err)
{
	uint32_t r = blockIdx.x * blockDim.x + threadIdx.x;
	if (r >= n_reads) return;
	uint64_t l = off[r + 1] - off[r];
	if (off[r + 1] < off[r] || l >= 0xfffffff0ull) { atomicOr(err, 1u); l = 0; }
	lens[r] = (uint32_t)l;
	words[r] = (uint32_t)(l / 32 + 1);
}

__device__ inline uint32_t base_code(uint8_t c, int ascii, uint32_t* bad)
{
	if (!ascii) { if (c > 4) *bad = 1; return c; }
	switch (c) { case 'A': return 0; case 'C': return 1; case 'G': return 2; case 'T': return 3; case 'N': return 4; }
	*bad = 1; return 4;
}

__global__ __launch_bounds__(256) void k_pack(const uint8_t* __restrict__ codes, const uint64_t* __restrict__ off,
                                              const uint64_t* __restrict__ word_off, const uint32_t* __restrict__ lens,
                                              uint32_t n_reads, int ascii, uint64_t* __restrict__ packed,
                                              uint32_t* __restrict__ inv, uint8_t* __restrict__ has_n, uint32_t* __restrict__ err)
{
	uint32_t r = blockIdx.x * 4 + (threadIdx.x >> 6);
	if (r >= n_reads) return;
	const uint32_t lane = threadIdx.x & 63;
	const uint32_t len = lens[r];
	const uint64_t src = off[r], wb = word_off[r];
	const uint32_t nw = len / 32 + 1;
	uint32_t bad = 0, anyn = 0;
	for (uint32_t w = lane; w < nw; w += 64)
	{
		uint64_t pw = 0; uint32_t iv = 0;
		uint32_t p0 = w * 32;
#pragma unroll 4
		for (uint32_t j = 0; j < 32; ++j)
		{
			uint32_t p = p0 + j;
			uint32_t c = 4; bool pad = p >= len;
			if (!pad) c = base_code(codes[src + p], ascii, &bad);
			if (c > 3) { iv |= 1u << (31 - j); if (!pad) anyn = 1; c = 0; }
			pw |= (uint64_t)c << (62 - 2 * j);
		}
		packed[wb + w] = pw; inv[wb + w] = iv;
	}
	uint64_t bn = __ballot(anyn != 0), bb = __ballot(bad != 0);
	if (lane == 0) { has_n[r] = bn != 0; if (bb) atomicOr(err, 2u); }
}

__global__ void k_arena_tail(uint64_t* packed, uint32_t* inv, uint64_t total_words)
{
	packed[total_words] = 0; inv[total_words] = 0xffffffffu;
}
}

extern "C" cl_status cl_reads_pack(cl_ctx* ctx, const uint8_t* d_codes, const uint64_t* d_offsets, uint32_t n_reads,
                                   int ascii, cl_reads** out)
{
	if (!ctx || !out || (!d_offsets)) return cl_fail(ctx, CL_E_INVALID, "cl_reads_pack: null argument");
	HIP_TRY(ctx, hipSetDevice(ctx->device));
	cl_reads* R = new cl_reads(); R->ctx = ctx; R->n_reads = n_reads;
	std::unique_ptr<cl_reads> guard(R);
	DEV_ALLOC(ctx, R->lens, n_reads); DEV_ALLOC(ctx, R->word_off, (uint64_t)n_reads + 1); DEV_ALLOC(ctx, R->has_n, n_reads);
	DevBuf<uint32_t> words; DEV_ALLOC(ctx, words, n_reads);
	DevBuf<uint32_t> err; DEV_ALLOC(ctx, err, 1);
	HIP_TRY(ctx, hipMemsetAsync(err.p, 0, 4, ctx->stream));
	if (n_reads)
	{
		LAUNCH(ctx, k_read_geometry, grid_for(n_reads, 256), 256, d_offsets, n_reads, R->lens.p, words.p, err.p);
		HIP_TRY(ctx, hipGetLastError());
	}
	CL_TRY(dev_exclusive_scan_u64(ctx, words.p, R->word_off.p, n_reads, &R->total_words));
	uint64_t first = 0, last = 0;
	if (n_reads)
	{
		HIP_TRY(ctx, hipMemcpyAsync(&first, d_offsets, 8, hipMemcpyDeviceToHost, ctx->stream));
		HIP_TRY(ctx, hipMemcpyAsync(&last, d_offsets + n_reads, 8, hipMemcpyDeviceToHost, ctx->stream));
		HIP_TRY(ctx, hipStreamSynchronize(ctx->stream));
	}
	R->total_bases = last - first;
	DEV_ALLOC(ctx, R->packed, R->total_words + 1); DEV_ALLOC(ctx, R->inv, R->total_words + 1);
	if (n_reads)
	{
		LAUNCH(ctx, k_pack, grid_for(n_reads, 4), 256, d_codes, d_offsets, (const uint64_t*)R->word_off.p,
			(const uint32_t*)R->lens.p, n_reads, ascii, R->packed.p, R->inv.p, R->has_n.p, err.p);
	}
	HIP_TRY(ctx, hipGetLastError());
	LAUNCH(ctx, k_arena_tail, 1, 1, R->packed.p, R->inv.p, R->total_words);
	uint32_t herr = 0;
	HIP_TRY(ctx, hipMemcpyAsync(&herr, err.p, 4, hipMemcpyDeviceToHost, ctx->stream));
	HIP_TRY(ctx, hipStreamSynchronize(ctx->stream));
	cl_timing_collect(ctx);
	if (herr & 1) return cl_fail(ctx, CL_E_INVALID, "cl_reads_pack: offsets not monotone or read too long");
	if (herr & 2) return cl_fail(ctx, CL_E_INVALID, "Only ACGTN symbols supported inside a read");
	*out = guard.release();
	return CL_OK;
}
extern "C" void cl_reads_free(cl_reads* r) { delete r; }
extern "C" uint32_t cl_reads_count(const cl_reads* r) { return r->n_reads; }
extern "C" uint64_t cl_reads_total_bases(const cl_reads* r) { return r->total_bases; }
extern "C" uint64_t cl_reads_total_words(const cl_reads* r) { return r->total_words; }
extern "C" const uint64_t* cl_reads_packed(const cl_reads* r) { return r->packed.p; }
extern "C" const uint32_t* cl_reads_invalid(const cl_reads* r) { return r->inv.p; }
extern "C" const uint64_t* cl_reads_word_offsets(const cl_reads* r) { return r->word_off.p; }
extern "C" const uint32_t* cl_reads_lengths(const cl_reads* r) { return r->lens.p; }
extern "C" const uint8_t* cl_reads_has_n(const cl_reads* r) { return r->has_n.p; }

namespace {
__global__ void k_select_geometry(const uint8_t* __restrict__ keep, const uint32_t* __restrict__ lens, uint32_t n, uint32_t* __restrict__ flag, uint32_t* __restrict__ words)
{
	const uint32_t i = blockIdx.x * blockDim.x + threadIdx.x;
	if (i >= n) return;
	const uint32_t kp = keep[i] ? 1u : 0u;
	flag[i] = kp; words[i] = kp ? lens[i] / 32 + 1 : 0u;
}
__global__ void k_select_copy(const uint8_t* __restrict__ keep, const uint32_t* __restrict__ rank, const uint64_t* __restrict__ new_off, const uint64_t* __restrict__ old_off,
                              const uint32_t* __restrict__ lens, const uint8_t* __restrict__ has_n, const uint64_t* __restrict__ packed, const uint32_t* __restrict__ inv, uint32_t n,
                              uint64_t* __restrict__ o_off, uint32_t* __restrict__ o_lens, uint8_t* __restrict__ o_has_n, uint64_t* __restrict__ o_packed, uint32_t* __restrict__ o_inv)
{
	const uint32_t r = (blockIdx.x * blockDim.x + threadIdx.x) >> 6, lane = threadIdx.x & 63;
	if (r >= n || !keep[r]) return;
	const uint32_t j = rank[r]; const uint64_t so = old_off[r], d = new_off[r]; const uint32_t w = lens[r] / 32 + 1;
	if (lane == 0) { o_off[j] = d; o_lens[j] = lens[r]; o_has_n[j] = has_n[r]; }
	for (uint32_t i = lane; i < w; i += 64) { o_packed[d + i] = packed[so + i]; o_inv[d + i] = inv[so + i]; }
}
}
extern "C" cl_status cl_reads_select(cl_ctx* ctx, const cl_reads* src, const uint8_t* d_keep, cl_reads** out)
{
	if (!ctx || !src || !d_keep || !out) return cl_fail(ctx, CL_E_INVALID, "cl_reads_select: null argument");
	HIP_TRY(ctx, hipSetDevice(ctx->device));
	const uint32_t n = src->n_reads;
	cl_reads* R = new cl_reads(); R->ctx = ctx;
	std::unique_ptr<cl_reads> guard(R);
	DevBuf<uint32_t> flag, words; DEV_ALLOC(ctx, flag, (uint64_t)n + 1); DEV_ALLOC(ctx, words, (uint64_t)n + 1);
	DevBuf<uint64_t> new_off; DEV_ALLOC(ctx, new_off, (uint64_t)n + 1);
	uint64_t kept = 0;
	if (n)
	{
		LAUNCH(ctx, k_select_geometry, grid_for(n, 256), 256, d_keep, (const uint32_t*)src->lens.p, n, flag.p, words.p);
		HIP_TRY(ctx, hipGetLastError());
	}
	CL_TRY(dev_exclusive_scan_u64(ctx, words.p, new_off.p, n, &R->total_words));
	CL_TRY(dev_exclusive_scan_u32(ctx, flag.p, n, &kept));
	R->n_reads = (uint32_t)kept;
	DEV_ALLOC(ctx, R->lens, kept); DEV_ALLOC(ctx, R->word_off, kept + 1); DEV_ALLOC(ctx, R->has_n, kept);
	DEV_ALLOC(ctx, R->packed, R->total_words + 1); DEV_ALLOC(ctx, R->inv, R->total_words + 1);
	if (n)
	{
		LAUNCHB(ctx, R->total_words * 24.0, k_select_copy, grid_for((uint64_t)n * 64, 256), 256, d_keep, (const uint32_t*)flag.p, (const uint64_t*)new_off.p, (const uint64_t*)src->word_off.p,
			(const uint32_t*)src->lens.p, (const uint8_t*)src->has_n.p, (const uint64_t*)src->packed.p, (const uint32_t*)src->inv.p, n,
			R->word_off.p, R->lens.p, R->has_n.p, R->packed.p, R->inv.p);
		HIP_TRY(ctx, hipGetLastError());
	}
	HIP_TRY(ctx, hipMemcpyAsync(R->word_off.p + kept, &R->total_words, 8, hipMemcpyHostToDevice, ctx->stream));
	LAUNCH(ctx, k_arena_tail, 1, 1, R->packed.p, R->inv.p, R->total_words);
	if (kept)
	{
		std::vector<uint32_t> h(kept);
		HIP_TRY(ctx, hipMemcpyAsync(h.data(), R->lens.p, kept * 4, hipMemcpyDeviceToHost, ctx->stream));
		HIP_TRY(ctx, hipStreamSynchronize(ctx->stream));
		uint64_t tb = 0; for (uint32_t l : h) tb += l;
		R->total_bases = tb;
	}
	HIP_TRY(ctx, hipStreamSynchronize(ctx->stream));
	cl_timing_collect(ctx);
	*out = guard.release();
	return CL_OK;
}

namespace {
__global__ void k_arena_geometry(const uint32_t* __restrict__ lens, uint32_t n, uint32_t* __restrict__ words)
{
	const uint32_t i = blockIdx.x * blockDim.x + threadIdx.x;
	if (i < n) words[i] = lens[i] / 32 + 1;
}
__global__ void k_arena_has_n(const uint64_t* __restrict__ off, const uint32_t* __restrict__ lens, const uint32_t* __restrict__ inv, uint32_t n, uint8_t* __restrict__ has_n)
{
	const uint32_t r = (blockIdx.x * blockDim.x + threadIdx.x) >> 6, lane = threadIdx.x & 63;
	if (r >= n) return;
	const uint32_t len = lens[r], w = len / 32 + 1; const uint64_t o = off[r];
	bool any = false;
	for (uint32_t i = lane; i < w; i += 64)
	{
		uint32_t m = inv[o + i];
		if (i == w - 1) m &= (len & 31) ? ~0u << (32 - (len & 31)) : 0u;
		any |= m != 0;
	}
	const uint64_t b = __ballot(any);
	if (lane == 0) has_n[r] = b ? 1 : 0;
}
}
extern "C" cl_status cl_reads_from_arena(cl_ctx* ctx, const uint64_t* d_packed, const uint32_t* d_inv, const uint32_t* d_lens, uint32_t n_reads, cl_reads** out)
{
	if (!ctx || !out || (n_reads && (!d_packed || !d_inv || !d_lens))) return cl_fail(ctx, CL_E_INVALID, "cl_reads_from_arena: null argument");
	HIP_TRY(ctx, hipSetDevice(ctx->device));
	cl_reads* R = new cl_reads(); R->ctx = ctx; R->n_reads = n_reads;
	std::unique_ptr<cl_reads> guard(R);
	DEV_ALLOC(ctx, R->lens, n_reads); DEV_ALLOC(ctx, R->word_off, (uint64_t)n_reads + 1); DEV_ALLOC(ctx, R->has_n, n_reads);
	DevBuf<uint32_t> words; DEV_ALLOC(ctx, words, (uint64_t)n_reads + 1);
	if (n_reads)
	{
		HIP_TRY(ctx, hipMemcpyAsync(R->lens.p, d_lens, (uint64_t)n_reads * 4, hipMemcpyDeviceToDevice, ctx->stream));
		LAUNCH(ctx, k_arena_geometry, grid_for(n_reads, 256), 256, d_lens, n_reads, words.p);
		HIP_TRY(ctx, hipGetLastError());
	}
	CL_TRY(dev_exclusive_scan_u64(ctx, words.p, R->word_off.p, n_reads, &R->total_words));
	DEV_ALLOC(ctx, R->packed, R->total_words + 1); DEV_ALLOC(ctx, R->inv, R->total_words + 1);
	if (R->total_words)
	{
		HIP_TRY(ctx, hipMemcpyAsync(R->packed.p, d_packed, R->total_words * 8, hipMemcpyDeviceToDevice, ctx->stream));
		HIP_TRY(ctx, hipMemcpyAsync(R->inv.p, d_inv, R->total_words * 4, hipMemcpyDeviceToDevice, ctx->stream));
	}
	LAUNCH(ctx, k_arena_tail, 1, 1, R->packed.p, R->inv.p, R->total_words);
	if (n_reads)
	{
		LAUNCH(ctx, k_arena_has_n, grid_for((uint64_t)n_reads * 64, 256), 256, (const uint64_t*)R->word_off.p, (const uint32_t*)R->lens.p, (const uint32_t*)R->inv.p, n_reads, R->has_n.p);
		HIP_TRY(ctx, hipGetLastError());
		std::vector<uint32_t> h(n_reads);
		HIP_TRY(ctx, hipMemcpyAsync(h.data(), R->lens.p, (uint64_t)n_reads * 4, hipMemcpyDeviceToHost, ctx->stream));
		HIP_TRY(ctx, hipStreamSynchronize(ctx->stream));
		uint64_t tb = 0; for (uint32_t l : h) tb += l;
		R->total_bases = tb;
	}
	HIP_TRY(ctx, hipStreamSynchronize(ctx->stream));
	cl_timing_collect(ctx);
	*out = guard.release();
	return CL_OK;
}

extern "C" cl_status cl_reads_compact(cl_ctx* ctx, const cl_reads* R, uint32_t read, uint8_t* h_out, uint64_t cap, uint64_t* n_out)
{
	if (!ctx || !R || read >= R->n_reads) return cl_fail(ctx, CL_E_INVALID, "cl_reads_compact: bad read index");
	uint32_t len = 0; uint64_t wo = 0;
	HIP_TRY(ctx, hipMemcpy(&len, R->lens.p + read, 4, hipMemcpyDeviceToHost));
	HIP_TRY(ctx, hipMemcpy(&wo, R->word_off.p + read, 8, hipMemcpyDeviceToHost));
	uint64_t nb = ((uint64_t)len + 3) / 4;
	if (n_out) *n_out = nb + 1;
	if (cap < nb + 1) return cl_fail(ctx, CL_E_CAPACITY, "cl_reads_compact: buffer too small");
	std::vector<uint64_t> w(len / 32 + 1);
	HIP_TRY(ctx, hipMemcpy(w.data(), R->packed.p + wo, w.size() * 8, hipMemcpyDeviceToHost));
	for (uint64_t b = 0; b < nb; ++b) h_out[b] = (uint8_t)(w[b / 8] >> (56 - 8 * (b % 8)));
	if (len % 4) h_out[nb - 1] &= (uint8_t)(0xff << (8 - 2 * (len % 4)));
	h_out[nb] = (uint8_t)(len % 4);
	return CL_OK;
}

namespace {

__device__ inline uint64_t revcomp_k(uint64_t x, uint32_t k)
{
	x = ~x;
	x = __brevll(x);
	x = ((x >> 1) & 0x5555555555555555ULL) | ((x & 0x5555555555555555ULL) << 1);
	return x >> (64 - 2 * k);
}
__device__ inline uint64_t fwd_at(uint64_t hi, uint64_t lo, uint32_t p, uint32_t k, uint64_t mask)
{
	uint32_t s = 128 - 2 * (p + k);
	uint64_t v = (s >= 64) ? (hi >> (s - 64)) : ((hi << (64 - s)) | (lo >> s));
	return v & mask;
}
__device__ inline bool window_valid(uint64_t inv64, uint32_t p, uint32_t k)
{
	return ((inv64 >> (64 - (p + k))) & ((1ULL << k) - 1)) == 0;
}

__device__ inline uint32_t scan_word(uint64_t hi, uint64_t lo, uint64_t inv64, uint32_t k, const ModTest& mt)
{
	if ((inv64 >> 32) == 0xffffffffull) return 0;
	const uint64_t mask = (1ULL << (2 * k)) - 1;
	const uint32_t roff = 2 * (k - 1);
	uint64_t fwd = hi >> (64 - 2 * k);
	uint64_t rev = revcomp_k(fwd, k);
	uint32_t res = 0;
#pragma unroll 8
	for (uint32_t p = 0; p < 32; ++p)
	{
		if (window_valid(inv64, p, k))
		{
			uint64_t can = fwd < rev ? fwd : rev;
			if (mod_is_zero(hash_mm(can), mt)) res |= 1u << p;
		}
		uint32_t j = p + k;
		uint64_t src = j < 32 ? hi : lo;
		uint64_t b = (src >> (62 - 2 * (j & 31))) & 3;
		fwd = ((fwd << 2) | b) & mask;
		rev = (rev >> 2) | ((3 - b) << roff);
	}
	return res;
}
__device__ inline uint64_t canonical_at(uint64_t hi, uint64_t lo, uint32_t p, uint32_t k)
{
	const uint64_t mask = (1ULL << (2 * k)) - 1;
	uint64_t f = fwd_at(hi, lo, p, k, mask);
	uint64_t r = revcomp_k(f, k);
	return f < r ? f : r;
}

__global__ __launch_bounds__(256) void k_kmer_scan(const uint64_t* __restrict__ packed, const uint32_t* __restrict__ inv,
                                                   uint64_t total_words, uint32_t k, ModTest mt,
                                                   uint64_t* __restrict__ out, uint64_t cap, unsigned long long* __restrict__ counter)
{
	__shared__ uint32_t sh[4];
	__shared__ unsigned long long sbase;
// ... 525 lines not shown
```

colord_amd/csrc/objects.hpp:

```cpp
#pragma once
#include "common.hpp"
#include <memory>

struct cl_reads {
	cl_ctx* ctx = nullptr;
	uint32_t n_reads = 0;
	uint64_t total_bases = 0, total_words = 0;
	DevBuf<uint64_t> packed;
	DevBuf<uint32_t> inv;
	DevBuf<uint64_t> word_off;
	DevBuf<uint32_t> lens;
	DevBuf<uint8_t> has_n;
};

struct cl_kmer_set {
	cl_ctx* ctx = nullptr;
	uint32_t k = 0;
	uint64_t n = 0;
	DevBuf<uint64_t> keys;
	DevBuf<uint32_t> counts;
	DevBuf<uint64_t> slots;
	uint64_t bmask = 0;
};

struct cl_kmer_lists {
	cl_ctx* ctx = nullptr;
	uint32_t n_reads = 0;
	uint64_t total = 0;
	DevBuf<uint64_t> off;
	DevBuf<uint64_t> kmers;
	DevBuf<uint32_t> ids;
	DevBuf<uint32_t> pos;
	DevBuf<uint32_t> read;
};

struct cl_index {
	cl_ctx* ctx = nullptr;
	uint32_t n_reads = 0, n_refs = 0, n_pseudo = 0;
	uint64_t n_keys = 0, n_entries = 0;
	DevBuf<uint32_t> ref_rank;
	DevBuf<uint64_t> off;
	DevBuf<uint32_t> refs;
};

uint32_t cl_part_shift(uint32_t k);
cl_status cl_key_histogram(cl_ctx* ctx, const uint64_t* d_kmers, uint64_t n, uint32_t k, std::vector<uint64_t>& h_bins);
cl_status cl_key_gather(cl_ctx* ctx, const uint64_t* d_kmers, uint64_t n, uint32_t k, uint32_t b0, uint32_t b1, uint64_t* d_out, uint64_t expect);

cl_status cl_ref_bounds(cl_ctx* ctx, const uint8_t* d_accept, uint32_t n, uint32_t ref_base, uint32_t* d_bounds, uint32_t* n_accepted);

cl_status cl_es_verify_at(cl_ctx* ctx, const cl_reads* reads, const cl_reads* refs, const uint8_t* d_es, const uint64_t* d_es_off, const uint32_t* d_es_ntuples,
                          uint64_t es_bytes, uint64_t* n_bad, uint32_t* first_bad, uint32_t* first_diff);

cl_status digest_chunk(cl_ctx* ctx, const cl_reads* reads, const cl_qual_params* qparams, const uint8_t* d_quals, const uint64_t* d_base_off, uint64_t first_read);
cl_status digest_values_chunk(cl_ctx* ctx, const cl_reads* reads, const cl_qual_params* qparams, const uint8_t* d_quals, const uint64_t* d_base_off, uint64_t first_read);
cl_status report_chunk(cl_ctx* ctx, const cl_reads* reads, const cl_qual_params* qparams, const uint8_t* d_quals, const uint64_t* d_base_off);
const cl_qual_params* cl_qual_coder_params(const cl_qual_coder* q);

#include <functional>
struct cl_dna_coder;
cl_status cl_dna_walk_ahead(cl_ctx* ctx, cl_dna_coder* D, const cl_reads* refs, const uint8_t* d_es, const uint64_t* d_es_off, const uint32_t* d_es_ntuples, uint32_t n_reads);
void cl_dna_set_before_tail(cl_dna_coder* D, std::function<cl_status()> fn);
struct DnaWalked;
cl_status cl_dna_prepare_batch(cl_ctx* ctx, cl_dna_coder* D, const cl_reads* refs, const uint8_t* d_es, const uint64_t* d_es_off, const uint32_t* d_es_ntuples, uint32_t n_reads,
                               uint32_t prev_types, uint32_t read_id, const uint32_t* h_part_bounds, uint32_t n_parts, DnaWalked** out, uint32_t* prev_types_out);
void cl_dna_walked_free(DnaWalked* W);
void cl_dna_set_ahead(cl_dna_coder* D, DnaWalked* W);
void cl_dna_coder_state(const cl_dna_coder* D, uint32_t* prev_types, uint32_t* read_id);
cl_status cl_dna_model_read(const cl_dna_coder* D, uint32_t family, uint64_t context, uint32_t* out);
cl_status cl_qual_model_read(const cl_qual_coder* Q, uint32_t family, uint64_t context, uint32_t* out, uint32_t cap, uint32_t* n_out);
cl_status cl_dna_batch_types(cl_ctx* ctx, const uint8_t* d_es, const uint64_t* d_es_off, uint32_t n_reads, uint64_t es_bytes, uint32_t prev_types, uint32_t* out);
struct QualPrepared;
cl_status cl_qual_prepare_batch(cl_ctx* ctx, cl_qual_coder* Q, const cl_reads* R, const uint8_t* d_quals, const uint64_t* d_qual_off,
                                const uint8_t* d_flags, const uint32_t* h_part_bounds, uint32_t n_parts, QualPrepared** out);
void cl_qual_prepared_free(QualPrepared* P);
void cl_qual_set_ahead(cl_qual_coder* Q, QualPrepared* P);
cl_status cl_dna_evolve_ahead(cl_ctx* ctx, cl_dna_coder* D, const cl_reads* refs, const uint8_t* d_es, const uint64_t* d_es_off, const uint32_t* d_es_ntuples, uint32_t n_reads,
                              const uint32_t* h_part_bounds, uint32_t n_parts, DnaWalked* W);
cl_status cl_qual_evolve_ahead(cl_ctx* ctx, cl_qual_coder* Q, const cl_reads* R, const uint8_t* d_quals, const uint64_t* d_qual_off, const uint32_t* h_part_bounds, uint32_t n_parts, QualPrepared* P);
void cl_qual_set_before_tail(cl_qual_coder* Q, std::function<cl_status()> fn);
constexpr cl_status CL_HOOK_RETRY = (cl_status)1000;
```

colord_amd/csrc/sort.hip:

```cpp
#include "common.hpp"
#include <string>

namespace {
constexpr uint32_t ST = 256;
constexpr uint32_t SI = 16;
constexpr uint32_t STILE = ST * SI;

template<typename K, uint32_t DB, uint32_t G>
__global__ __launch_bounds__(ST) void k_sort_hist(const K* __restrict__ keys, uint64_t n, uint32_t shift, uint32_t dmask,
                                                  uint32_t* __restrict__ hist, uint32_t nb)
{
	constexpr uint32_t ND = 1u << DB;
	constexpr uint32_t ROW = G > 1 ? ND + 1 : ND;
	__shared__ uint32_t h[G * ROW];
	for (uint32_t i = threadIdx.x; i < G * ROW; i += ST) h[i] = 0;
	__syncthreads();
	const uint32_t tile0 = blockIdx.x * G;
	for (uint32_t g = 0; g < G && tile0 + g < nb; ++g)
	{
		const uint64_t base = (uint64_t)(tile0 + g) * STILE;
#pragma unroll
		for (uint32_t i = 0; i < SI; ++i)
		{
			uint64_t idx = base + (uint64_t)i * ST + threadIdx.x;
			if (idx < n) atomicAdd(&h[g * ROW + ((uint32_t)(keys[idx] >> shift) & dmask)], 1u);
		}
	}
	__syncthreads();
	for (uint32_t i = threadIdx.x; i < G * ND; i += ST)
	{
		const uint32_t g = i % G, d = i / G;
		if (tile0 + g < nb) hist[(uint64_t)d * nb + tile0 + g] = h[g * ROW + d];
	}
}

template<typename K, bool HAS_V, uint32_t DB>
__global__ __launch_bounds__(ST) void k_sort_scatter(const K* __restrict__ kin, const uint32_t* __restrict__ vin,
                                                     K* __restrict__ kout, uint32_t* __restrict__ vout,
                                                     uint64_t n, uint32_t shift, uint32_t dmask, const uint32_t* __restrict__ offs, uint32_t nb)
{
	constexpr uint32_t ND = 1u << DB, PER = ND / ST;
	__shared__ uint32_t wh[4][ND];
	__shared__ uint32_t lstart[ND + 1];
	__shared__ uint32_t gdelta[ND];
	__shared__ uint32_t wtot[4];
	__shared__ K skey[STILE];
	__shared__ uint32_t sval[HAS_V ? STILE : 1];
	const uint32_t w = threadIdx.x >> 6, lane = threadIdx.x & 63;
	for (uint32_t i = threadIdx.x; i < 4 * ND; i += ST) (&wh[0][0])[i] = 0;
	__syncthreads();

	const uint64_t tbase = (uint64_t)blockIdx.x * STILE, wbase = tbase + (uint64_t)w * (64 * SI);
	K key[SI]; uint32_t rank[SI]; uint32_t val[HAS_V ? SI : 1];
	const uint64_t lt = (1ULL << lane) - 1;
	uint32_t goff[PER];
#pragma unroll
	for (uint32_t k = 0; k < PER; ++k) goff[k] = offs[(uint64_t)(threadIdx.x * PER + k) * nb + blockIdx.x];
#pragma unroll
	for (uint32_t r = 0; r < SI; ++r)
	{
		uint64_t idx = wbase + (uint64_t)r * 64 + lane;
		key[r] = idx < n ? kin[idx] : (K)0;
		if (HAS_V) val[r] = idx < n ? vin[idx] : 0u;
	}
#pragma unroll
	for (uint32_t r = 0; r < SI; ++r)
	{
		uint64_t idx = wbase + (uint64_t)r * 64 + lane;
		bool valid = idx < n;
		uint32_t d = (uint32_t)(key[r] >> shift) & dmask;
		uint64_t peers = __ballot(valid);
#pragma unroll
		for (uint32_t b = 0; b < DB; ++b)
		{
			bool bit = (d >> b) & 1u;
			uint64_t m = __ballot(valid && bit);
			peers &= bit ? m : ~m;
		}
		uint32_t prior = valid ? wh[w][d] : 0u;
		rank[r] = prior + (uint32_t)__popcll(peers & lt);
		__builtin_amdgcn_wave_barrier();
		if (valid && (peers & lt) == 0) wh[w][d] = prior + (uint32_t)__popcll(peers);
		__builtin_amdgcn_wave_barrier();
	}
	__syncthreads();
	{
		uint32_t c[PER][4], tot[PER], mine = 0;
#pragma unroll
		for (uint32_t k = 0; k < PER; ++k)
		{
			const uint32_t d = threadIdx.x * PER + k;
			c[k][0] = wh[0][d]; c[k][1] = wh[1][d]; c[k][2] = wh[2][d]; c[k][3] = wh[3][d];
			tot[k] = c[k][0] + c[k][1] + c[k][2] + c[k][3]; mine += tot[k];
		}
		uint32_t incl = mine;
#pragma unroll
		for (uint32_t o = 1; o < 64; o <<= 1) { const uint32_t t = __shfl_up(incl, o, 64); if (lane >= o) incl += t; }
		if (lane == 63) wtot[w] = incl;
		__syncthreads();
		uint32_t ls = incl - mine;
		for (uint32_t i = 0; i < w; ++i) ls += wtot[i];
#pragma unroll
		for (uint32_t k = 0; k < PER; ++k)
		{
			const uint32_t d = threadIdx.x * PER + k;
			lstart[d] = ls;
			if (d == ND - 1) lstart[ND] = ls + tot[k];
			gdelta[d] = goff[k] - ls;
			wh[0][d] = ls; wh[1][d] = ls + c[k][0]; wh[2][d] = ls + c[k][0] + c[k][1]; wh[3][d] = ls + c[k][0] + c[k][1] + c[k][2];
			ls += tot[k];
		}
	}
	__syncthreads();
#pragma unroll
	for (uint32_t r = 0; r < SI; ++r)
	{
		uint64_t idx = wbase + (uint64_t)r * 64 + lane;
		if (idx < n)
		{
			uint32_t d = (uint32_t)(key[r] >> shift) & dmask;
			uint32_t lp = wh[w][d] + rank[r];
			skey[lp] = key[r];
			if (HAS_V) sval[lp] = val[r];
		}
	}
	__syncthreads();
	const uint32_t tile_n = lstart[ND];
	for (uint32_t j = threadIdx.x; j < tile_n; j += ST)
	{
		const K k = skey[j];
		const uint32_t pos = gdelta[(uint32_t)(k >> shift) & dmask] + j;
		kout[pos] = k;
		if (HAS_V) vout[pos] = sval[j];
	}
}

template<typename K, uint32_t DB>
cl_status sort_pass(cl_ctx* ctx, const K* kin, const uint32_t* vin, K* kout, uint32_t* vout, uint64_t n, uint32_t shift, uint32_t dmask, uint32_t* hist, uint32_t nb)
{
	static const std::string kt = sizeof(K) == 8 ? "unsigned long" : "unsigned int", db = std::to_string(DB) + "u";
	constexpr uint32_t G = DB == 8 ? 16 : 4; const bool grouped = nb >= 4096;
	static const std::string n_hist1 = "k_sort_hist<" + kt + ", " + db + ", 1u>", n_histg = "k_sort_hist<" + kt + ", " + db + ", " + std::to_string(G) + "u>", n_sv = "k_sort_scatter<" + kt + ", true, " + db + ">", n_sk = "k_sort_scatter<" + kt + ", false, " + db + ">";
	if (grouped) LAUNCHB_NAMED(ctx, n_histg.c_str(), n * sizeof(K), (k_sort_hist<K, DB, G>), (nb + G - 1) / G, ST, kin, n, shift, dmask, hist, nb);
	else LAUNCHB_NAMED(ctx, n_hist1.c_str(), n * sizeof(K), (k_sort_hist<K, DB, 1>), nb, ST, kin, n, shift, dmask, hist, nb);
	HIP_TRY(ctx, hipGetLastError());
	CL_TRY(dev_exclusive_scan_u32(ctx, hist, (uint64_t)(1u << DB) * nb, nullptr));
	if (vin) LAUNCHB_NAMED(ctx, n_sv.c_str(), n * (2 * sizeof(K) + 8), (k_sort_scatter<K, true, DB>), nb, ST, kin, vin, kout, vout, n, shift, dmask, (const uint32_t*)hist, nb);
	else LAUNCHB_NAMED(ctx, n_sk.c_str(), n * 2 * sizeof(K), (k_sort_scatter<K, false, DB>), nb, ST, kin, (const uint32_t*)nullptr, kout, (uint32_t*)nullptr, n, shift, dmask, (const uint32_t*)hist, nb);
	HIP_TRY(ctx, hipGetLastError());
	return CL_OK;
}

template<typename K>
cl_status sort_impl(cl_ctx* ctx, K* d_keys, uint32_t* d_vals, uint64_t n, uint32_t begin_bit, uint32_t end_bit, DevBuf<K>* swap_k = nullptr, DevBuf<uint32_t>* swap_v = nullptr)
{
	if (end_bit > 8 * sizeof(K)) return cl_fail(ctx, CL_E_INVALID, "radix sort: end_bit " + std::to_string(end_bit) + " is beyond the key's " + std::to_string(8 * sizeof(K)) + " bits");
	if (n <= 1 || end_bit <= begin_bit) return CL_OK;
	if (n >= (1ULL << 32)) return cl_fail(ctx, CL_E_UNSUPPORTED, "radix sort: n must be < 2^32 per call");
	const uint32_t nb = grid_for(n, STILE);
	const uint32_t bits = end_bit - begin_bit;
	const uint32_t n_pass_real = (bits + 7) / 8 == (bits + 9) / 10 ? (bits + 7) / 8 : (bits + 9) / 10;
	const uint32_t db_hi = (bits + n_pass_real - 1) / n_pass_real;
	const bool third = (n_pass_real & 1) && n_pass_real > 1 && n * (sizeof(K) + (d_vals ? 4 : 0)) <= (2ull << 30);
	const uint32_t n_pass = third ? n_pass_real : (n_pass_real + 1) & ~1u;
	DevBuf<K> ktmp, ktmp2; DEV_ALLOC(ctx, ktmp, n);
	DevBuf<uint32_t> vtmp, vtmp2; if (d_vals) DEV_ALLOC(ctx, vtmp, n);
	if (n_pass & 1) { DEV_ALLOC(ctx, ktmp2, n); if (d_vals) DEV_ALLOC(ctx, vtmp2, n); }
	DevBuf<uint32_t> hist; DEV_ALLOC(ctx, hist, (uint64_t)(1u << std::max(8u, db_hi)) * nb);
	K* kin = d_keys; uint32_t* vin = d_vals;
	uint32_t pass = 0;
	for (uint32_t shift = begin_bit; shift < end_bit; ++pass)
	{
		K* kout; uint32_t* vout;
		if (n_pass & 1) { kout = pass == 0 ? ktmp2.p : (pass & 1) ? ktmp.p : d_keys; vout = pass == 0 ? vtmp2.p : (pass & 1) ? vtmp.p : d_vals; }
		else { kout = (pass & 1) ? d_keys : ktmp.p; vout = (pass & 1) ? d_vals : vtmp.p; }
		const uint32_t left = end_bit - shift, passes_left = n_pass_real - pass;
		const uint32_t db = std::max(8u, (left + passes_left - 1) / passes_left);
		const uint32_t use = std::min(db, 10u);
		const uint32_t dmask = (1u << std::min(use, left)) - 1;
		if (use == 10) CL_TRY((sort_pass<K, 10>(ctx, kin, vin, kout, vout, n, shift, dmask, hist.p, nb)));
		else if (use == 9) CL_TRY((sort_pass<K, 9>(ctx, kin, vin, kout, vout, n, shift, dmask, hist.p, nb)));
		else CL_TRY((sort_pass<K, 8>(ctx, kin, vin, kout, vout, n, shift, dmask, hist.p, nb)));
		shift += use;
		kin = kout; vin = vout;
	}
	if (kin != d_keys && swap_k && kin == ktmp.p && (!d_vals || (swap_v && vin == vtmp.p)))
	{
		std::swap(*swap_k, ktmp);
		if (d_vals) std::swap(*swap_v, vtmp);
	}
	else if (kin != d_keys)
	{
		HIP_TRY(ctx, hipMemcpyAsync(d_keys, kin, n * sizeof(K), hipMemcpyDeviceToDevice, cl_launch_stream(ctx)));
		if (d_vals) HIP_TRY(ctx, hipMemcpyAsync(d_vals, vin, n * 4, hipMemcpyDeviceToDevice, cl_launch_stream(ctx)));
	}
	HIP_TRY(ctx, hipStreamSynchronize(cl_launch_stream(ctx)));
	return CL_OK;
}
}

cl_status dev_sort_pairs(cl_ctx* ctx, uint64_t* d_keys, uint32_t* d_vals, uint64_t n, uint32_t begin_bit, uint32_t end_bit)
{
	return sort_impl<uint64_t>(ctx, d_keys, d_vals, n, begin_bit, end_bit);
}
cl_status dev_sort_pairs_swap(cl_ctx* ctx, DevBuf<uint64_t>& keys, DevBuf<uint32_t>& vals, uint64_t n, uint32_t begin_bit, uint32_t end_bit)
{
	if (keys.n != n || vals.n != n) return sort_impl<uint64_t>(ctx, keys.p, vals.p, n, begin_bit, end_bit);
	return sort_impl<uint64_t>(ctx, keys.p, vals.p, n, begin_bit, end_bit, &keys, &vals);
}
cl_status dev_sort_keys32_pairs(cl_ctx* ctx, uint32_t* d_keys, uint32_t* d_vals, uint64_t n, uint32_t begin_bit, uint32_t end_bit)
{
	return sort_impl<uint32_t>(ctx, d_keys, d_vals, n, begin_bit, end_bit);
}
cl_status dev_sort_keys32_pairs_swap(cl_ctx* ctx, DevBuf<uint32_t>& keys, DevBuf<uint32_t>& vals, uint64_t n, uint32_t begin_bit, uint32_t end_bit)
{
	if (keys.n != n || vals.n != n) return sort_impl<uint32_t>(ctx, keys.p, vals.p, n, begin_bit, end_bit);
	return sort_impl<uint32_t>(ctx, keys.p, vals.p, n, begin_bit, end_bit, &keys, &vals);
}
```

colord_amd/device.py:

```python
from __future__ import annotations
import ctypes as C
import numpy as np
import torch
from . import _native as N


def _check(ctx, st):
    if ctx is not None and getattr(ctx, "timing", False):
        for n, (ms, k, b, cells) in ctx.kernel_times().items():
            a = ctx.acc.setdefault(n, [0.0, 0, 0.0, 0.0])
            a[0] += ms
            a[1] += k
            a[2] += b
            a[3] += cells
    if st != N.CL_OK:
        msg = N.load().cl_last_error(ctx.h).decode() if ctx is not None and ctx.h else ""
        raise N.ColordHipError(st, msg)


def _view(ptr, n, dtype, device):
    out = torch.empty(int(n), dtype=dtype, device=device)
    if n:
        torch.cuda.synchronize(device)
        rc = _hip().hipMemcpy(C.c_void_p(out.data_ptr()), C.c_void_p(ptr), C.c_size_t(int(n) * out.element_size()), 3)
        if rc != 0:
            raise N.ColordHipError(N.CL_E_HIP, f"hipMemcpy failed ({rc})")
    return out


_HIP = None


def _hip():
    global _HIP
    if _HIP is None:
        _HIP = C.CDLL("libamdhip64.so")
        _HIP.hipMemcpy.argtypes = [C.c_void_p, C.c_void_p, C.c_size_t, C.c_int]
        _HIP.hipMemcpy.restype = C.c_int
    return _HIP


class _OrderedLib:
    _HOST_ONLY = ("cl_last_error", "cl_ctx_kernel_times", "cl_ctx_last_kernel_ms", "cl_ctx_set_timing", "cl_ref_accept", "cl_ctx_set_verify", "cl_ctx_verified",
                  "cl_compressor_verified", "cl_ctx_set_verify_streams", "cl_ctx_verified_streams", "cl_compressor_verified_streams",
                  "cl_ctx_set_digest", "cl_ctx_digest", "cl_compressor_digest", "cl_digest_bases_host", "cl_digest_bytes_host", "cl_qual_decoder_set_digest", "cl_qual_decoder_digest",
                  "cl_ctx_set_digest_values", "cl_ctx_digest_values", "cl_compressor_digest_values", "cl_qual_values_host", "cl_digest_qual_values_host",
                  "cl_qual_coder_domains", "cl_compressor_qual_domains", "cl_ctx_gap_paths",
                  "cl_report_clear", "cl_report_add", "cl_report_bases_host", "cl_report_quals_host", "cl_report_values_host", "cl_ctx_set_report", "cl_ctx_report", "cl_compressor_report")

    def __init__(self, lib, device):
        self._lib, self._device, self._cache = lib, device, {}

    def __getattr__(self, name):
        f = self._cache.get(name)
        if f is None:
            raw = getattr(self._lib, name)
            if not name.startswith("cl_") or name in self._HOST_ONLY or name.endswith("_free") or name.endswith("_destroy"):
                f = raw
            else:
                dev = self._device

                def f(*a, _raw=raw, _dev=dev):
                    torch.cuda.current_stream(_dev).synchronize()
                    return _raw(*a)
            self._cache[name] = f
        return f


class Context:
    def __init__(self, device: int = 0, timing: bool = False):
        self.lib = N.load()
        if not torch.cuda.is_available():
            raise N.ColordHipError(N.CL_E_HIP, "no GPU visible: the HIP path cannot run (no CPU fallback)")
        self.h = N._P()
        st = self.lib.cl_ctx_create(device, C.byref(self.h))
        if st != N.CL_OK:
            raise N.ColordHipError(st, "cl_ctx_create failed")
        self.device = torch.device("cuda", device)
        self.lib = _OrderedLib(self.lib, self.device)
        self.timing = timing
        self.acc = {}
        if timing:
            self.lib.cl_ctx_set_timing(self.h, 1)

    def close(self):
        if self.h:
            self.lib.cl_ctx_destroy(self.h)
            self.h = None

    def kernel_ms(self, name: str):
        ms, n = C.c_double(0), C.c_uint32(0)
        self.lib.cl_ctx_last_kernel_ms(self.h, name.encode(), C.byref(ms), C.byref(n))
        return ms.value, n.value

    def kernel_times(self) -> dict:
        buf = C.create_string_buffer(1 << 16)
        need = C.c_uint64(0)
        if self.lib.cl_ctx_kernel_times(self.h, buf, len(buf), C.byref(need)) != N.CL_OK:
            return {}
        out = {}
        for line in buf.value.decode().splitlines():
            f = line.split("\t")
            out[f[0]] = (float(f[1]), int(f[2]), float(f[3]), float(f[4]) if len(f) > 4 else 0.0)
        return out

    def set_verify(self, on: bool = True):
        self.lib.cl_ctx_set_verify(self.h, int(bool(on)))

    def verified(self):
        r, b = C.c_uint64(0), C.c_uint64(0)
        _check(None, self.lib.cl_ctx_verified(self.h, C.byref(r), C.byref(b)))
        return r.value, b.value

    def gap_paths(self):
        out = (C.c_uint64 * 11)()
        _check(None, self.lib.cl_ctx_gap_paths(self.h, out, 11))
        v = [int(x) for x in out]
        return {"classes": v[:8], "quad_to_wave": v[8], "giant_to_wave": v[9], "wave_redo_rounds": v[10]}

    def set_verify_streams(self, on: bool = True):
        self.lib.cl_ctx_set_verify_streams(self.h, int(bool(on)))

    def verified_streams(self):
        p, s, b = C.c_uint64(0), C.c_uint64(0), C.c_uint64(0)
        _check(None, self.lib.cl_ctx_verified_streams(self.h, C.byref(p), C.byref(s), C.byref(b)))
        return p.value, s.value, b.value

    def set_digest(self, on: bool = True):
        self.lib.cl_ctx_set_digest(self.h, int(bool(on)))

    def digest(self):
        d, q = N.Digest(), N.Digest()
        _check(None, self.lib.cl_ctx_digest(self.h, C.byref(d), C.byref(q)))
        return d.triple(), q.triple()

    def digest_bases(self, reads: "Reads", first_read: int = 0, acc: "N.Digest | None" = None):
        acc = N.Digest() if acc is None else acc
        _check(self, self.lib.cl_digest_bases(self.h, reads.h, first_read, C.byref(acc)))
        return acc.triple()

    def digest_quals(self, reads: "Reads", quals: torch.Tensor, qual_off: torch.Tensor, mode: int, fwd=(), first_read: int = 0, acc: "N.Digest | None" = None):
        prm = N.QualParams()
        prm.mode, prm.source, prm.level, prm.n_fwd = mode, 0, 1, len(fwd)
        for i, v in enumerate(fwd):
            prm.fwd[i] = v
        acc = N.Digest() if acc is None else acc
        quals, qual_off = quals.contiguous(), qual_off.contiguous()
        _check(self, self.lib.cl_digest_quals(self.h, C.byref(prm), reads.h, quals.data_ptr() if quals.numel() else None, qual_off.data_ptr(), first_read, C.byref(acc)))
        return acc.triple()

    def set_digest_values(self, on: bool = True):
        self.lib.cl_ctx_set_digest_values(self.h, int(bool(on)))

    def digest_values(self):
        d = N.Digest()
        _check(None, self.lib.cl_ctx_digest_values(self.h, C.byref(d)))
        return d.triple()

    def set_report(self, on: bool = True):
        self.lib.cl_ctx_set_report(self.h, int(bool(on)))

    def report(self) -> "N.Report":
        r = N.Report()
        _check(None, self.lib.cl_ctx_report(self.h, C.byref(r)))
        return r

    @staticmethod
    def new_report() -> "N.Report":
        r = N.Report()
        N.load().cl_report_clear(C.byref(r))
        return r

    def report_bases(self, reads: "Reads", acc: "N.Report | None" = None) -> "N.Report":
        acc = self.new_report() if acc is None else acc
        _check(self, self.lib.cl_report_bases(self.h, reads.h, C.byref(acc)))
        return acc

    def report_quals(self, reads: "Reads", quals: torch.Tensor, qual_off: torch.Tensor, mode: int, fwd=(), rev=(), flush_bytes: int = 0, max_blocks: int = 0,
                     acc: "N.Report | None" = None) -> "N.Report":
        prm = self._qual_params(mode, fwd, rev)
        acc = self.new_report() if acc is None else acc
        quals, qual_off = quals.contiguous(), qual_off.contiguous()
        _check(self, self.lib.cl_report_quals(self.h, C.byref(prm), reads.h, quals.data_ptr() if quals.numel() else None, qual_off.data_ptr(), flush_bytes, max_blocks, C.byref(acc)))
        return acc

    @staticmethod
    def _qual_params(mode, fwd, rev):
        prm = N.QualParams()
        prm.mode, prm.source, prm.level, prm.n_fwd, prm.n_rev = mode, 0, 1, len(fwd), len(rev)
        for i, v in enumerate(fwd):
            prm.fwd[i] = v
        for i, v in enumerate(rev):
            prm.rev[i] = v
        return prm

    def digest_qual_values(self, reads: "Reads", quals: torch.Tensor, qual_off: torch.Tensor, mode: int, fwd=(), rev=(), first_read: int = 0, acc: "N.Digest | None" = None):
        prm = self._qual_params(mode, fwd, rev)
        acc = N.Digest() if acc is None else acc
        quals, qual_off = quals.contiguous(), qual_off.contiguous()
        _check(self, self.lib.cl_digest_qual_values(self.h, C.byref(prm), reads.h, quals.data_ptr() if quals.numel() else None, qual_off.data_ptr(), first_read, C.byref(acc)))
        return acc.triple()
# ... 250 lines not shown
        P = N.CompressParams()
        for k_, v in params.items():
            setattr(P, k_, v)
        pb = np.ascontiguousarray(np.asarray(part_bounds, dtype=np.uint32)); kb = np.ascontiguousarray(np.asarray(pack_bounds, dtype=np.uint32))
        npart = len(pb) - 1
        dcap = int(reads.total_bases) + 64 * npart + 4096
        dout = torch.empty(dcap, dtype=torch.uint8, device=self.device)
        dsz = np.zeros(max(npart, 1), np.uint64)
        qout, qsz, qcap = None, np.zeros(max(npart, 1), np.uint64), 0
        if qual is not None:
            qcap = int(int(reads.total_bases) * 1.35) + 64 * npart + 4096
            qout = torch.empty(qcap, dtype=torch.uint8, device=self.device)
        info = N.CompressInfo()
        _check(self, self.lib.cl_compress_shard(self.h, C.byref(P), reads.h, quals.data_ptr() if qual is not None else None,
                                                base_off.contiguous().data_ptr() if qual is not None else None,
                                                pb.ctypes.data, npart, kb.ctypes.data, len(kb) - 1, dna.h, qual.h if qual is not None else None,
                                                dout.data_ptr(), dcap, dsz.ctypes.data, qout.data_ptr() if qout is not None else None, qcap, qsz.ctypes.data, C.byref(info)))
        if qual is not None and qual.ctx is not self:
            _check(qual.ctx, N.CL_OK)
        inf = {n_: getattr(info, n_) for n_, _ in N.CompressInfo._fields_ if n_ != "pad"}
        return dout[:inf["dna_bytes"]], dsz[:npart], (qout[:inf["qual_bytes"]] if qout is not None else None), qsz[:npart], inf

    def compressor(self, params: dict, qual_params=None, qual_ctx: "Context | None" = None, exchange=None, expected_bases: int = 0) -> "Compressor":
        P = N.CompressParams()
        for k_, v in params.items():
            setattr(P, k_, v)
        Q = None
        if qual_params is not None:
            mode, source, level, fwd, rev = qual_params
            Q = N.QualParams(mode=mode, source=source, level=level, n_fwd=len(fwd), n_rev=len(rev))
            for i, v in enumerate(fwd):
                Q.fwd[i] = v
            for i, v in enumerate(rev):
                Q.rev[i] = v
        h = N._P()
        _check(self, self.lib.cl_compressor_create(self.h, qual_ctx.h if qual_ctx is not None else None, C.byref(P), C.byref(Q) if Q is not None else None,
                                                   C.byref(exchange.c_struct) if exchange is not None else None, int(expected_bases), C.byref(h)))
        return Compressor(self, h, qual_ctx, Q is not None, exchange)

    def dna_coder(self, max_alt_refs: int, level: int, start_read_id: int = 0) -> "DnaCoder":
        h = N._P()
        _check(self, self.lib.cl_dna_coder_create(self.h, max_alt_refs, level, start_read_id, C.byref(h)))
        return DnaCoder(self, h, max_alt_refs)

    def sort_u64(self, keys: torch.Tensor, vals: torch.Tensor | None = None, begin_bit=0, end_bit=64):
        if vals is None:
            _check(self, self.lib.cl_sort_u64(self.h, keys.data_ptr(), keys.numel(), begin_bit, end_bit))
        else:
            _check(self, self.lib.cl_sort_u64_u32(self.h, keys.data_ptr(), vals.data_ptr(), keys.numel(), begin_bit, end_bit))

    def sort_u32(self, keys: torch.Tensor, vals: torch.Tensor | None = None, begin_bit=0, end_bit=32):
        assert keys.dtype == torch.int32 and (vals is None or vals.dtype == torch.int32)
        if vals is None:
            _check(self, self.lib.cl_sort_u32(self.h, keys.data_ptr(), keys.numel(), begin_bit, end_bit))
        else:
            _check(self, self.lib.cl_sort_u32_u32(self.h, keys.data_ptr(), vals.data_ptr(), keys.numel(), begin_bit, end_bit))

    def sort_swap(self, keys: torch.Tensor, vals: torch.Tensor, begin_bit, end_bit):
        assert keys.dtype in (torch.int32, torch.int64) and vals.dtype == torch.int32 and vals.numel() == keys.numel()
        ko, vo = torch.empty_like(keys), torch.empty_like(vals)
        f = self.lib.cl_sort_swap_u32_u32 if keys.dtype == torch.int32 else self.lib.cl_sort_swap_u64_u32
        _check(self, f(self.h, keys.data_ptr(), vals.data_ptr(), keys.numel(), begin_bit, end_bit, ko.data_ptr(), vo.data_ptr()))
        return ko, vo

    def scan_u32(self, data: torch.Tensor, want_total: bool = True):
        assert data.dtype == torch.int32
        total = C.c_uint64(0)
        _check(self, self.lib.cl_scan_u32(self.h, data.data_ptr(), data.numel(), C.byref(total) if want_total else None))
        return total.value if want_total else None

    def scan_u32_u64(self, data: torch.Tensor, out: torch.Tensor, want_total: bool = True):
        assert data.dtype == torch.int32 and out.dtype == torch.int64 and out.numel() == data.numel() + 1
        total = C.c_uint64(0)
        _check(self, self.lib.cl_scan_u32_u64(self.h, data.data_ptr(), out.data_ptr(), data.numel(), C.byref(total) if want_total else None))
        return total.value if want_total else None

    def run_starts(self, keys: torch.Tensor, shift: int, seg: torch.Tensor) -> int:
        assert keys.dtype in (torch.int32, torch.int64) and seg.dtype == torch.int32
        f = self.lib.cl_run_starts_u32 if keys.dtype == torch.int32 else self.lib.cl_run_starts_u64
        r = C.c_uint64(0)
        _check(self, f(self.h, keys.data_ptr(), keys.numel(), shift, seg.data_ptr(), seg.numel(), C.byref(r)))
        return r.value


class _Obj:
    _free = None

    def __init__(self, ctx, h):
        self.ctx, self.h = ctx, h

    def free(self):
        if self.h:
            getattr(self.ctx.lib, self._free)(self.h)
            self.h = None

    def _arr(self, getter, n, dtype):
        ptr = getattr(self.ctx.lib, getter)(self.h)
        return _view(ptr, n, dtype, self.ctx.device)


class Reads(_Obj):
    _free = "cl_reads_free"

    @property
    def n_reads(self): return self.ctx.lib.cl_reads_count(self.h)
    @property
    def total_bases(self): return self.ctx.lib.cl_reads_total_bases(self.h)
    @property
    def total_words(self): return self.ctx.lib.cl_reads_total_words(self.h)
    def packed(self): return self._arr("cl_reads_packed", self.total_words + 1, torch.int64)
    def invalid(self): return self._arr("cl_reads_invalid", self.total_words + 1, torch.int32)
    def word_offsets(self): return self._arr("cl_reads_word_offsets", self.n_reads + 1, torch.int64)
    def lengths(self): return self._arr("cl_reads_lengths", self.n_reads, torch.int32)
    def has_n(self): return self._arr("cl_reads_has_n", self.n_reads, torch.uint8)

    def compact(self, i: int) -> bytes:
        buf = np.zeros(1 << 20, np.uint8)
        n = C.c_uint64(0)
        st = self.ctx.lib.cl_reads_compact(self.ctx.h, self.h, i, buf.ctypes.data, buf.size, C.byref(n))
        if st == N.CL_E_CAPACITY:
            buf = np.zeros(n.value, np.uint8)
            st = self.ctx.lib.cl_reads_compact(self.ctx.h, self.h, i, buf.ctypes.data, buf.size, C.byref(n))
        _check(self.ctx, st)
        return bytes(buf[:n.value])


class KmerSet(_Obj):
    _free = "cl_kmer_set_free"

    @property
    def size(self): return self.ctx.lib.cl_kmer_set_size(self.h)
    def keys(self): return self._arr("cl_kmer_set_keys", self.size, torch.int64)
    def counts(self): return self._arr("cl_kmer_set_counts", self.size, torch.int32)

    def check(self, kmers: torch.Tensor) -> torch.Tensor:
        out = torch.empty(kmers.numel(), dtype=torch.uint8, device=self.ctx.device)
        _check(self.ctx, self.ctx.lib.cl_kmer_set_check(self.ctx.h, self.h, kmers.data_ptr(), kmers.numel(), out.data_ptr()))
        return out


class KmerLists(_Obj):
    _free = "cl_kmer_lists_free"

    @property
    def n_reads(self): return self.ctx.lib.cl_kmer_lists_reads(self.h)
    @property
    def total(self): return self.ctx.lib.cl_kmer_lists_total(self.h)
    def offsets(self): return self._arr("cl_kmer_lists_offsets", self.n_reads + 1, torch.int64)
    def kmers(self): return self._arr("cl_kmer_lists_kmers", self.total, torch.int64)
    def ids(self): return self._arr("cl_kmer_lists_ids", self.total, torch.int32)
    def pos(self): return self._arr("cl_kmer_lists_pos", self.total, torch.int32)


class Index(_Obj):
    _free = "cl_index_free"

    @property
    def n_refs(self): return self.ctx.lib.cl_index_n_refs(self.h)
    @property
    def entries(self): return self.ctx.lib.cl_index_entries(self.h)


class QualCoder(_Obj):
    _free = "cl_qual_coder_free"

    def encode(self, reads: "Reads", quals: torch.Tensor, qual_off: torch.Tensor, part_bounds, flags: torch.Tensor | None = None):
# ... 179 lines not shown
```

include/colord_hip.h:

```cpp
#ifndef COLORD_HIP_H
#define COLORD_HIP_H
#include <stdint.h>
#include <stddef.h>

#ifdef __cplusplus
extern "C" {
#endif

typedef int32_t cl_status;
enum {
	CL_OK = 0,
	CL_E_INVALID = -1,
	CL_E_HIP = -2,
	CL_E_CAPACITY = -3,
	CL_E_NOMEM = -4,
	CL_E_UNSUPPORTED = -5,
	CL_E_MISMATCH = -6
};

typedef struct cl_ctx cl_ctx;
typedef struct cl_reads cl_reads;
typedef struct cl_kmer_set cl_kmer_set;
typedef struct cl_kmer_lists cl_kmer_lists;
typedef struct cl_index cl_index;

cl_status cl_ctx_create(int device, cl_ctx** out);
void cl_ctx_destroy(cl_ctx* ctx);
const char* cl_last_error(const cl_ctx* ctx);
void* cl_ctx_stream(cl_ctx* ctx);
cl_status cl_ctx_last_kernel_ms(const cl_ctx* ctx, const char* kernel, double* ms, uint32_t* launches);
cl_status cl_ctx_kernel_times(cl_ctx* ctx, char* buf, uint64_t cap, uint64_t* needed);
void cl_ctx_set_timing(cl_ctx* ctx, int on);
void cl_ctx_set_verify(cl_ctx* ctx, int on);
cl_status cl_ctx_verified(const cl_ctx* ctx, uint64_t* reads, uint64_t* bases);
void cl_ctx_set_verify_streams(cl_ctx* ctx, int on);
cl_status cl_ctx_verified_streams(const cl_ctx* ctx, uint64_t* parts, uint64_t* symbols, uint64_t* bytes);
cl_status cl_ctx_gap_paths(const cl_ctx* ctx, uint64_t* out, uint32_t cap);
typedef struct cl_digest { uint64_t reads, symbols, sum; } cl_digest;
void cl_ctx_set_digest(cl_ctx* ctx, int on);
cl_status cl_ctx_digest(const cl_ctx* ctx, cl_digest* dna, cl_digest* qual);
void cl_ctx_set_digest_values(cl_ctx* ctx, int on);
cl_status cl_ctx_digest_values(const cl_ctx* ctx, cl_digest* out);

cl_status cl_reads_pack(cl_ctx* ctx, const uint8_t* d_codes, const uint64_t* d_offsets, uint32_t n_reads,
                        int ascii, cl_reads** out);
void cl_reads_free(cl_reads* r);
uint32_t cl_reads_count(const cl_reads* r);
uint64_t cl_reads_total_bases(const cl_reads* r);
uint64_t cl_reads_total_words(const cl_reads* r);
const uint64_t* cl_reads_packed(const cl_reads* r);
const uint32_t* cl_reads_invalid(const cl_reads* r);
const uint64_t* cl_reads_word_offsets(const cl_reads* r);
const uint32_t* cl_reads_lengths(const cl_reads* r);
const uint8_t* cl_reads_has_n(const cl_reads* r);

cl_status cl_kmer_scan(cl_ctx* ctx, const cl_reads* reads, uint32_t k, uint32_t f,
                       uint64_t* d_out, uint64_t cap, uint64_t* n_out);

typedef struct {
	uint64_t n_reads;
	uint64_t tot_kmers;
	uint64_t n_unique;
	uint64_t n_unique_counted;
	uint64_t total_count_filtered;
} cl_kmer_stats;
cl_status cl_kmer_count_filter(cl_ctx* ctx, uint64_t* d_kmers, uint64_t n, uint32_t k, uint32_t ci, uint32_t cs,
                               cl_kmer_set** out, cl_kmer_stats* stats);
cl_status cl_kmer_set_create(cl_ctx* ctx, const uint64_t* d_keys, const uint32_t* d_counts, uint64_t n, uint32_t k, cl_kmer_set** out);
void cl_kmer_set_free(cl_kmer_set* s);
uint64_t cl_kmer_set_size(const cl_kmer_set* s);
const uint64_t* cl_kmer_set_keys(const cl_kmer_set* s);
const uint32_t* cl_kmer_set_counts(const cl_kmer_set* s);
cl_status cl_kmer_set_check(cl_ctx* ctx, const cl_kmer_set* s, const uint64_t* d_kmers, uint64_t n, uint8_t* d_found);

cl_status cl_accepted_kmers(cl_ctx* ctx, const cl_kmer_set* set, const cl_reads* reads, uint32_t k, uint32_t f,
                            cl_kmer_lists** out);
void cl_kmer_lists_free(cl_kmer_lists* l);
uint32_t cl_kmer_lists_reads(const cl_kmer_lists* l);
uint64_t cl_kmer_lists_total(const cl_kmer_lists* l);
const uint64_t* cl_kmer_lists_offsets(const cl_kmer_lists* l);
const uint64_t* cl_kmer_lists_kmers(const cl_kmer_lists* l);
const uint32_t* cl_kmer_lists_ids(const cl_kmer_lists* l);
const uint32_t* cl_kmer_lists_pos(const cl_kmer_lists* l);

cl_status cl_ref_accept(uint32_t n_reads, uint32_t n_pseudo, uint32_t range, double exponent, uint8_t* h_out);

cl_status cl_index_build(cl_ctx* ctx, const cl_kmer_set* set, const cl_kmer_lists* lists, const uint8_t* d_accept,
                         uint32_t n_pseudo, uint32_t max_kmer_count, cl_index** out);
cl_status cl_index_entries_of(cl_ctx* ctx, const cl_kmer_lists* lists, const uint8_t* d_accept, uint32_t ref_base,
                              uint32_t* d_ids, uint32_t* d_refs, uint64_t cap, uint64_t* n_out,
                              uint32_t* d_bounds, uint32_t* n_accepted);
cl_status cl_index_build_pairs(cl_ctx* ctx, const cl_kmer_set* set, uint32_t* d_ids, uint32_t* d_refs, uint64_t n,
                               const uint32_t* d_bounds, uint32_t n_reads, uint32_t n_refs_total,
                               uint32_t n_pseudo, uint32_t max_kmer_count, cl_index** out);
void cl_index_free(cl_index* ix);
uint32_t cl_index_n_refs(const cl_index* ix);
uint64_t cl_index_entries(const cl_index* ix);
const uint32_t* cl_index_ref_rank(const cl_index* ix);
cl_status cl_candidates(cl_ctx* ctx, const cl_index* ix, const cl_kmer_lists* lists, uint32_t max_candidates,
                        uint32_t* d_refs, uint32_t* d_votes, uint32_t* d_n);
cl_status cl_candidates_at(cl_ctx* ctx, const cl_index* ix, const cl_kmer_lists* lists, const uint32_t* d_bounds, uint32_t max_candidates,
                           uint32_t* d_refs, uint32_t* d_votes, uint32_t* d_n);
cl_status cl_candidates_common(cl_ctx* ctx, const cl_index* ix, const cl_kmer_lists* lists, uint32_t max_candidates,
                               const uint32_t* d_refs, const uint32_t* d_n,
                               uint64_t* d_common_off, uint64_t* d_common, uint64_t cap, uint64_t* n_common);

typedef struct cl_qual_coder cl_qual_coder;
typedef struct {
	int32_t mode;
	int32_t source;
	int32_t level;
	uint32_t n_fwd;
	uint32_t fwd[8];
	uint32_t n_rev;
	uint32_t rev[8];
} cl_qual_params;
cl_status cl_qual_coder_create(cl_ctx* ctx, const cl_qual_params* params, cl_qual_coder** out);
void cl_qual_coder_free(cl_qual_coder* q);
cl_ctx* cl_qual_coder_ctx(const cl_qual_coder* q);
cl_status cl_qual_encode(cl_ctx* ctx, cl_qual_coder* q, const cl_reads* reads, const uint8_t* d_quals, const uint64_t* d_qual_off,
// ... 99 lines not shown
                            uint8_t* d_dna_out, uint64_t dna_cap, uint64_t* h_dna_part_sizes,
                            uint8_t* d_qual_out, uint64_t qual_cap, uint64_t* h_qual_part_sizes, cl_compress_info* info);

typedef struct cl_compressor cl_compressor;
typedef struct {
	void* user;
	uint32_t rank, world;
	cl_status (*all_gather_host)(void* user, const uint64_t* h_vals, uint32_t n, uint64_t* h_out);
	cl_status (*all_to_all_v)(void* user, const void* d_send, const uint64_t* h_send_bytes, void* d_recv, const uint64_t* h_recv_bytes);
	cl_status (*all_gather_v)(void* user, const void* d_send, uint64_t send_bytes, void* d_recv, const uint64_t* h_recv_bytes);
} cl_exchange;
cl_status cl_compressor_create(cl_ctx* ctx, cl_ctx* qual_ctx, const cl_compress_params* params, const cl_qual_params* qparams,
                               const cl_exchange* exchange, uint64_t expected_bases, cl_compressor** out);
void cl_compressor_free(cl_compressor* c);
cl_status cl_compressor_count_add(cl_compressor* c, const cl_reads* chunk);
cl_status cl_compressor_count_finish(cl_compressor* c, cl_kmer_stats* stats);
cl_status cl_compressor_refs_add(cl_compressor* c, const cl_reads* chunk);
cl_status cl_compressor_refs_finish(cl_compressor* c);
cl_status cl_compressor_encode(cl_compressor* c, const cl_reads* chunk, const uint8_t* d_quals, const uint64_t* d_base_off,
                               const uint32_t* h_part_bounds, uint32_t n_parts, const uint32_t* h_pack_bounds, uint32_t n_packs,
                               uint8_t* d_dna_out, uint64_t dna_cap, uint64_t* h_dna_part_sizes,
                               uint8_t* d_qual_out, uint64_t qual_cap, uint64_t* h_qual_part_sizes, cl_compress_info* info);
cl_status cl_compressor_genome_add(cl_compressor* c, const cl_reads* sequences);
cl_status cl_compressor_pseudo_reads(cl_compressor* c, const cl_reads* pseudo_reads);
cl_status cl_compressor_prepare(cl_compressor* c, const cl_reads* chunk, const uint32_t* h_pack_bounds, uint32_t n_packs);
cl_status cl_compressor_prepare_parts(cl_compressor* c, const cl_reads* chunk, const uint32_t* h_pack_bounds, uint32_t n_packs, const uint32_t* h_part_bounds, uint32_t n_parts,
                                      const uint8_t* d_quals, const uint64_t* d_base_off);
cl_status cl_compressor_info(const cl_compressor* c, cl_kmer_stats* stats, uint64_t* first_read, uint64_t* n_reads_total, uint64_t* mean_read_len,
                             uint32_t* sparse_range, uint32_t* n_refs_total);
cl_status cl_compressor_verified(const cl_compressor* c, uint64_t* reads, uint64_t* bases);
cl_status cl_compressor_verified_streams(const cl_compressor* c, uint64_t* parts, uint64_t* symbols, uint64_t* bytes);
cl_status cl_compressor_digest(const cl_compressor* c, cl_digest* dna, cl_digest* qual);
cl_status cl_compressor_digest_values(const cl_compressor* c, cl_digest* out);
cl_status cl_compressor_report(const cl_compressor* c, cl_report* out);

cl_status cl_compressor_set_qual_domain_symbols(cl_compressor* c, uint64_t n);
cl_status cl_compressor_qual_domains(const cl_compressor* c, uint64_t* h_first_part, uint64_t cap, uint64_t* n_out);

cl_status cl_genome_encode(const uint8_t* h_codes, const uint64_t* h_off, uint32_t n_seqs, uint8_t* h_out, uint64_t cap, uint64_t* n_out);
cl_status cl_genome_decode(const uint8_t* h_in, uint64_t n_in, uint32_t n_seqs, uint8_t* h_codes, uint64_t cap, uint64_t* h_off, uint64_t* n_out);
cl_status cl_genome_md5(const uint8_t* h_codes, const uint64_t* h_off, uint32_t n_seqs, uint8_t* h_md5_16);

typedef struct cl_dna_decoder cl_dna_decoder;
typedef struct cl_qual_decoder cl_qual_decoder;
typedef struct cl_id_decoder cl_id_decoder;
cl_status cl_dna_decoder_create(uint32_t max_alt_refs, int32_t level, uint32_t start_read_id, uint32_t n_pseudo,
                                int32_t accept_all, uint32_t sparse_range, double sparse_exponent, cl_dna_decoder** out);
void cl_dna_decoder_free(cl_dna_decoder* d);
const char* cl_dna_decoder_error(const cl_dna_decoder* d);
cl_status cl_dna_decoder_add_ref(cl_dna_decoder* d, const uint8_t* h_codes, uint32_t len);
cl_status cl_dna_decoder_new_domain(cl_dna_decoder* d);
cl_status cl_dna_decode_part(cl_dna_decoder* d, const uint8_t* h_in, uint64_t n_in, uint32_t n_reads,
                             uint8_t* h_bases, uint64_t cap, uint64_t* h_off, uint64_t* n_out);
cl_status cl_qual_decoder_create(const cl_qual_params* params, cl_qual_decoder** out);
void cl_qual_decoder_free(cl_qual_decoder* q);
cl_status cl_qual_decoder_new_domain(cl_qual_decoder* q);
cl_status cl_qual_decode_part(cl_qual_decoder* q, const uint8_t* h_in, uint64_t n_in, const uint8_t* h_bases, const uint64_t* h_off,
                              uint32_t n_reads, uint8_t* h_quals);
cl_status cl_qual_decoder_set_digest(cl_qual_decoder* q, int on, uint64_t first_read);
cl_status cl_qual_decoder_digest(const cl_qual_decoder* q, cl_digest* out);
cl_status cl_qual_decode_domains(cl_ctx* ctx, const cl_qual_params* params, const cl_reads* reads, const uint8_t* d_flags,
                                 const uint8_t* d_in, uint64_t n_in, const uint32_t* h_part_bounds, const uint64_t* h_part_sizes, uint32_t n_parts,
                                 const uint32_t* h_domain_first_part, uint32_t n_domains, uint32_t max_domains_per_launch,
                                 uint8_t* d_quals, const uint64_t* d_qual_off, uint64_t quals_cap, uint8_t* d_symbols, uint64_t symbols_cap);
cl_status cl_id_decoder_create(int32_t header_mode, cl_id_decoder** out);
void cl_id_decoder_free(cl_id_decoder* c);
cl_status cl_id_decode_part(cl_id_decoder* c, const uint8_t* h_in, uint64_t n_in, uint32_t n, uint8_t* h_ids, uint64_t cap,
                            uint64_t* h_off, uint8_t* h_plus, uint64_t* n_out);

cl_status cl_reads_compact(cl_ctx* ctx, const cl_reads* reads, uint32_t read, uint8_t* h_out, uint64_t cap, uint64_t* n_out);

cl_status cl_sort_u64(cl_ctx* ctx, uint64_t* d_keys, uint64_t n, uint32_t begin_bit, uint32_t end_bit);
cl_status cl_sort_u64_u32(cl_ctx* ctx, uint64_t* d_keys, uint32_t* d_vals, uint64_t n, uint32_t begin_bit, uint32_t end_bit);
cl_status cl_sort_u32(cl_ctx* ctx, uint32_t* d_keys, uint64_t n, uint32_t begin_bit, uint32_t end_bit);
cl_status cl_sort_u32_u32(cl_ctx* ctx, uint32_t* d_keys, uint32_t* d_vals, uint64_t n, uint32_t begin_bit, uint32_t end_bit);
cl_status cl_sort_swap_u32_u32(cl_ctx* ctx, const uint32_t* d_keys_in, const uint32_t* d_vals_in, uint64_t n, uint32_t begin_bit, uint32_t end_bit,
                               uint32_t* d_keys_out, uint32_t* d_vals_out);
cl_status cl_sort_swap_u64_u32(cl_ctx* ctx, const uint64_t* d_keys_in, const uint32_t* d_vals_in, uint64_t n, uint32_t begin_bit, uint32_t end_bit,
                               uint64_t* d_keys_out, uint32_t* d_vals_out);
cl_status cl_scan_u32(cl_ctx* ctx, uint32_t* d_data, uint64_t n, uint64_t* h_total);
cl_status cl_scan_u32_u64(cl_ctx* ctx, const uint32_t* d_in, uint64_t* d_out, uint64_t n, uint64_t* h_total);
cl_status cl_run_starts_u32(cl_ctx* ctx, const uint32_t* d_keys, uint64_t n, uint32_t shift, uint32_t* d_seg, uint64_t seg_cap, uint64_t* h_n_runs);
cl_status cl_run_starts_u64(cl_ctx* ctx, const uint64_t* d_keys, uint64_t n, uint32_t shift, uint32_t* d_seg, uint64_t seg_cap, uint64_t* h_n_runs);

#ifdef __cplusplus
}
#endif
#endif
```

Before: 2.997.

## Replace full anchor pair radix sort with high-bit sort plus segmented tie sorting

In the anchor candidate stage, the full radix sort over pe+pr+tb bits is replaced by a radix sort over only the high (pe+tb) bits. Runs of equal high keys are then fixed up by a per-thread insertion sort for short runs and a block-level bitonic sort in LDS for runs up to 2048 keys. Runs that are too long fall back to the full sort. Separately, max read length is now tracked at pack time, which drops a device-to-host copy of reference lengths per call. The change adds tie-fixup kernels and a host slot readback, and it costs a second full sort whenever a fallback occurs.

```diff
diff --git a/colord_amd/_native.py b/colord_amd/_native.py
--- a/colord_amd/_native.py
+++ b/colord_amd/_native.py
@@ -80,6 +80,7 @@
     "cl_ctx_set_verify": (None, [_P, C.c_int]),
     "cl_ctx_verified": (C.c_int32, [_P, C.POINTER(C.c_uint64), C.POINTER(C.c_uint64)]),
     "cl_ctx_gap_paths": (C.c_int32, [_P, C.POINTER(C.c_uint64), C.c_uint32]),
+    "cl_ctx_pair_sort_stats": (C.c_int32, [_P, C.POINTER(C.c_uint64), C.c_uint32]),
     "cl_ctx_set_verify_streams": (None, [_P, C.c_int]),
     "cl_ctx_verified_streams": (C.c_int32, [_P, C.POINTER(C.c_uint64), C.POINTER(C.c_uint64), C.POINTER(C.c_uint64)]),
     "cl_compressor_verified_streams": (C.c_int32, [_P, C.POINTER(C.c_uint64), C.POINTER(C.c_uint64), C.POINTER(C.c_uint64)]),
@@ -224,6 +225,7 @@
     "cl_scan_u32_u64": (C.c_int32, [_P, _P, _P, C.c_uint64, C.POINTER(C.c_uint64)]),
     "cl_run_starts_u32": (C.c_int32, [_P, _P, C.c_uint64, C.c_uint32, _P, C.c_uint64, C.POINTER(C.c_uint64)]),
     "cl_run_starts_u64": (C.c_int32, [_P, _P, C.c_uint64, C.c_uint32, _P, C.c_uint64, C.POINTER(C.c_uint64)]),
+    "cl_pair_sort_u64": (C.c_int32, [_P, _P, C.c_uint64, C.c_uint32, C.c_uint32, C.POINTER(C.c_uint64)]),
 }
 
 _lib = None
diff --git a/colord_amd/csrc/anchors.hip b/colord_amd/csrc/anchors.hip
--- a/colord_amd/csrc/anchors.hip
+++ b/colord_amd/csrc/anchors.hip
@@ -792,17 +792,15 @@
 	std::unique_ptr<cl_anchors> guard(X);
 	DEV_ALLOC(ctx, X->n_cands, nr); DEV_ALLOC(ctx, X->cand, (uint64_t)nr * c * 4); DEV_ALLOC(ctx, X->cand_off, (uint64_t)nr * c + 1);
 	Arena A{ reads->packed.p, reads->word_off.p, reads->lens.p }, R{ refs->packed.p, refs->word_off.p, refs->lens.p };
+	const bool stamp = getenv("COLORD_HIP_STREAM_DEBUG") != nullptr;
+	const auto t_call = std::chrono::steady_clock::now();
+	auto ms_since = [&](std::chrono::steady_clock::time_point t) { return std::chrono::duration<double, std::milli>(std::chrono::steady_clock::now() - t).count(); };
+	double ms_lens = 0, ms_prepare = 0;
 	std::vector<uint32_t> h_len(nr);
 	if (nr) HIP_TRY(ctx, hipMemcpy(h_len.data(), reads->lens.p, (uint64_t)nr * 4, hipMemcpyDeviceToHost));
 	auto bits_for = [](uint64_t v) -> uint32_t { uint32_t b = 1; while ((1ull << b) <= v) ++b; return b; };
-	uint32_t max_ref_len = 0;
-	if (refs->n_reads)
-	{
-		std::vector<uint32_t> rl(refs->n_reads);
-		HIP_TRY(ctx, hipMemcpy(rl.data(), refs->lens.p, (uint64_t)refs->n_reads * 4, hipMemcpyDeviceToHost));
-		for (uint32_t l : rl) max_ref_len = std::max(max_ref_len, l);
-	}
-	const uint32_t pr_bits = bits_for(max_ref_len);
+	const uint32_t pr_bits = bits_for(refs->max_len);
+	ms_lens = ms_since(t_call);
 	const uint64_t BATCH_BASES = 1ull << 28;
 	std::vector<DevBuf<uint32_t>> chunks; std::vector<uint64_t> chunk_n;
 	uint64_t total_anchors = 0;
@@ -858,6 +856,8 @@
 	};
 	std::unique_ptr<TableBatch> cur, nxt;
 	if (nr) CL_TRY(prepare(0, cur));
+	ms_prepare = ms_since(t_call);
+	bool first_batch = true;
 	while (cur)
 	{
 		const uint32_t r0 = cur->r0, r1 = cur->r1; const uint64_t acc = cur->acc;
@@ -866,6 +866,10 @@
 		HIP_TRY(ctx, hipStreamSynchronize(ctx->stream));
 		HIP_TRY(ctx, hipStreamSynchronize(ctx->side));
 		cur->sync.s = nullptr;
+		if (stamp && first_batch)
+			fprintf(stderr, "[stream] anchors call, %u reads, %u references: read lengths on the host after %.2f ms, first batch's tables queued after %.2f ms, built after %.2f ms (the main stream's first match pass follows)\n",
+				nr, refs->n_reads, ms_lens, ms_prepare, ms_since(t_call));
+		first_batch = false;
 		{ uint32_t herr = 0; HIP_TRY(ctx, hipMemcpy(&herr, cur->err.p, 4, hipMemcpyDeviceToHost)); if (herr) return cl_fail(ctx, CL_E_UNSUPPORTED, "cl_anchor_candidates: a region of an m-mer table overflowed"); }
 		DevBuf<uint32_t>& n_distinct = cur->n_distinct;
 		EncTable T{ cur->slots.p, cur->toff.p, cur->next.p, cur->noff.p };
@@ -905,7 +909,15 @@
 		if (n_pairs)
 		{
 			uint32_t tb = 1; while ((1ull << tb) < n_tasks) ++tb;
-			CL_TRY(dev_sort_pairs(ctx, pairs.p, nullptr, n_pairs, 0, cfg.pe + cfg.pr + tb));
+			PairSortStats ps;
+			CL_TRY(dev_pair_sort(ctx, pairs.p, n_pairs, cfg.pr, cfg.pe + tb, &ps));
+			if (getenv("COLORD_HIP_ANCHOR_DEBUG"))
+			{
+				const PairSortStats& T = ctx->pair_sort;
+				fprintf(stderr, "[anchors] pair sort tb %u pe %u pr %u: pairs %llu runs %llu to blocks %llu fallback %llu full %llu | context total: calls %llu pairs %llu runs %llu to blocks %llu fallbacks %llu full %llu\n",
+					tb, cfg.pe, cfg.pr, (unsigned long long)ps.pairs, (unsigned long long)ps.runs, (unsigned long long)ps.block_runs, (unsigned long long)ps.fallbacks, (unsigned long long)ps.full,
+					(unsigned long long)T.calls, (unsigned long long)T.pairs, (unsigned long long)T.runs, (unsigned long long)T.block_runs, (unsigned long long)T.fallbacks, (unsigned long long)T.full);
+			}
 		}
 		LAUNCH(ctx, k_task_pairs, grid_for((uint64_t)n_tasks + 1, 256), 256, (const uint64_t*)pairs.p, n_pairs, A, cfg, (const uint32_t*)n_distinct.p, n_tasks, pair_off.p, pair_cnt.p);
 		LAUNCHB(ctx, n_pairs * 32.0, k_lis_anchors, grid_for(n_tasks, 64), 64, A, R, cfg, d_cand_refs, n_tasks, (const uint64_t*)pair_off.p, (const uint32_t*)pair_cnt.p, (const uint64_t*)pairs.p,
diff --git a/colord_amd/csrc/capi.hip b/colord_amd/csrc/capi.hip
--- a/colord_amd/csrc/capi.hip
+++ b/colord_amd/csrc/capi.hip
@@ -130,6 +130,14 @@
 	for (uint32_t i = 0; i < cap && i < 11; ++i) out[i] = c->gap_paths[i];
 	return CL_OK;
 }
+extern "C" cl_status cl_ctx_pair_sort_stats(const cl_ctx* c, uint64_t* out, uint32_t cap)
+{
+	if (!c || (!out && cap)) return CL_E_INVALID;
+	const PairSortStats& T = c->pair_sort;
+	const uint64_t v[8] = { T.calls, T.pairs, T.runs, T.block_runs, T.fallbacks, T.full, T.pr, T.hi };
+	for (uint32_t i = 0; i < cap && i < 8; ++i) out[i] = v[i];
+	return CL_OK;
+}
 extern "C" cl_status cl_dna_coder_model(const cl_dna_coder* d, uint32_t family, uint64_t context, uint32_t* out)
 {
 	if (!d || !out) return CL_E_INVALID;
@@ -245,6 +253,21 @@
 	cl_status s = dev_run_starts_u64(ctx, d_keys, n, shift, d_seg, seg_cap, h_n_runs);
 	cl_timing_collect(ctx);
 	return s;
+}
+extern "C" cl_status cl_pair_sort_u64(cl_ctx* ctx, uint64_t* d_keys, uint64_t n, uint32_t pr_bits, uint32_t hi_bits, uint64_t* h_stats)
+{
+	if (!ctx || !h_stats || (!d_keys && n)) return cl_fail(ctx, CL_E_INVALID, "cl_pair_sort_u64: null argument");
+	HIP_TRY(ctx, hipSetDevice(ctx->device));
+	cl_timing_begin(ctx);
+	PairSortStats S;
+	cl_status s = dev_pair_sort(ctx, d_keys, n, pr_bits, hi_bits, &S);
+	hipError_t e = hipStreamSynchronize(ctx->stream);
+	cl_timing_collect(ctx);
+	if (s == CL_OK) HIP_TRY(ctx, e);
+	if (s != CL_OK) return s;
+	const uint64_t out[8] = { S.pairs, S.runs, S.block_runs, S.fallbacks, S.full, S.pr, S.hi, ctx->pair_sort.calls };
+	memcpy(h_stats, out, sizeof out);
+	return CL_OK;
 }
 extern "C" cl_status cl_sort_u32(cl_ctx* ctx, uint32_t* d_keys, uint64_t n, uint32_t begin_bit, uint32_t end_bit)
 {
diff --git a/colord_amd/csrc/common.hpp b/colord_amd/csrc/common.hpp
--- a/colord_amd/csrc/common.hpp
+++ b/colord_amd/csrc/common.hpp
@@ -18,6 +18,7 @@
 #include <condition_variable>
 #include <thread>
 #include <chrono>
+#include <functional>
 #include "../../include/colord_hip.h"
 
 #define CL_WAVE 64
@@ -290,6 +291,10 @@
 	if (--it->second.second == 0) it->second.first->trim();
 }
 
+struct PairSortStats {
+	uint64_t calls = 0, pairs = 0, runs = 0, block_runs = 0, fallbacks = 0, full = 0; uint32_t pr = 0, hi = 0;
+	void add(const PairSortStats& o) { ++calls; pairs += o.pairs; runs += o.runs; block_runs += o.block_runs; fallbacks += o.fallbacks; full += o.full; pr = o.pr; hi = o.hi; }
+};
 struct cl_ctx {
 	DevPool& pool;
 	int device = 0;
@@ -315,6 +320,7 @@
 	cl_digest digest_qval{ 0, 0, 0 };
 	bool report = false;
 	cl_report* report_acc = nullptr;
+	PairSortStats pair_sort;
 	uint64_t gap_paths[11] = { 0 };
 	std::map<std::string, KernelTime> times;
 	std::vector<std::pair<std::string, std::pair<hipEvent_t, hipEvent_t>>> pending;
@@ -570,6 +576,8 @@
 cl_status dev_run_starts_u32(cl_ctx* ctx, const uint32_t* d_keys, uint64_t n, uint32_t shift, uint32_t* d_seg, uint64_t seg_cap, uint64_t* h_n_runs);
 cl_status dev_run_starts_u64(cl_ctx* ctx, const uint64_t* d_keys, uint64_t n, uint32_t shift, uint32_t* d_seg, uint64_t seg_cap, uint64_t* h_n_runs);
 cl_status dev_sort_pairs(cl_ctx* ctx, uint64_t* d_keys, uint32_t* d_vals, uint64_t n, uint32_t begin_bit, uint32_t end_bit);
+cl_status dev_sort_pairs_then(cl_ctx* ctx, uint64_t* d_keys, uint64_t n, uint32_t begin_bit, uint32_t end_bit, const std::function<cl_status()>& after);
+cl_status dev_pair_sort(cl_ctx* ctx, uint64_t* d_keys, uint64_t n, uint32_t pr_bits, uint32_t hi_bits, PairSortStats* st);
 cl_status dev_sort_pairs_swap(cl_ctx* ctx, DevBuf<uint64_t>& keys, DevBuf<uint32_t>& vals, uint64_t n, uint32_t begin_bit, uint32_t end_bit);
 cl_status dev_sort_keys32_pairs(cl_ctx* ctx, uint32_t* d_keys, uint32_t* d_vals, uint64_t n, uint32_t begin_bit, uint32_t end_bit);
 cl_status dev_sort_keys32_pairs_swap(cl_ctx* ctx, DevBuf<uint32_t>& keys, DevBuf<uint32_t>& vals, uint64_t n, uint32_t begin_bit, uint32_t end_bit);
diff --git a/colord_amd/csrc/kmer.hip b/colord_amd/csrc/kmer.hip
--- a/colord_amd/csrc/kmer.hip
+++ b/colord_amd/csrc/kmer.hip
@@ -14,6 +14,7 @@
 	if (off[r + 1] < off[r] || l >= 0xfffffff0ull) { atomicOr(err, 1u); l = 0; }
 	lens[r] = (uint32_t)l;
 	words[r] = (uint32_t)(l / 32 + 1);
+	atomicMax(err + 1, (uint32_t)l);
 }
 
 __device__ inline uint32_t base_code(uint8_t c, int ascii, uint32_t* bad)
@@ -69,8 +70,8 @@
 	std::unique_ptr<cl_reads> guard(R);
 	DEV_ALLOC(ctx, R->lens, n_reads); DEV_ALLOC(ctx, R->word_off, (uint64_t)n_reads + 1); DEV_ALLOC(ctx, R->has_n, n_reads);
 	DevBuf<uint32_t> words; DEV_ALLOC(ctx, words, n_reads);
-	DevBuf<uint32_t> err; DEV_ALLOC(ctx, err, 1);
-	HIP_TRY(ctx, hipMemsetAsync(err.p, 0, 4, ctx->stream));
+	DevBuf<uint32_t> err; DEV_ALLOC(ctx, err, 2);
+	HIP_TRY(ctx, hipMemsetAsync(err.p, 0, 8, ctx->stream));
 	if (n_reads)
 	{
 		LAUNCH(ctx, k_read_geometry, grid_for(n_reads, 256), 256, d_offsets, n_reads, R->lens.p, words.p, err.p);
@@ -93,10 +94,12 @@
 	}
 	HIP_TRY(ctx, hipGetLastError());
 	LAUNCH(ctx, k_arena_tail, 1, 1, R->packed.p, R->inv.p, R->total_words);
-	uint32_t herr = 0;
-	HIP_TRY(ctx, hipMemcpyAsync(&herr, err.p, 4, hipMemcpyDeviceToHost, ctx->stream));
+	uint32_t herr2[2] = { 0, 0 };
+	HIP_TRY(ctx, hipMemcpyAsync(herr2, err.p, 8, hipMemcpyDeviceToHost, ctx->stream));
 	HIP_TRY(ctx, hipStreamSynchronize(ctx->stream));
 	cl_timing_collect(ctx);
+	const uint32_t herr = herr2[0];
+	R->max_len = herr2[1];
 	if (herr & 1) return cl_fail(ctx, CL_E_INVALID, "cl_reads_pack: offsets not monotone or read too long");
 	if (herr & 2) return cl_fail(ctx, CL_E_INVALID, "Only ACGTN symbols supported inside a read");
 	*out = guard.release();
@@ -165,7 +168,7 @@
 		std::vector<uint32_t> h(kept);
 		HIP_TRY(ctx, hipMemcpyAsync(h.data(), R->lens.p, kept * 4, hipMemcpyDeviceToHost, ctx->stream));
 		HIP_TRY(ctx, hipStreamSynchronize(ctx->stream));
-		uint64_t tb = 0; for (uint32_t l : h) tb += l;
+		uint64_t tb = 0; for (uint32_t l : h) { tb += l; R->max_len = std::max(R->max_len, l); }
 		R->total_bases = tb;
 	}
 	HIP_TRY(ctx, hipStreamSynchronize(ctx->stream));
@@ -225,7 +228,7 @@
 		std::vector<uint32_t> h(n_reads);
 		HIP_TRY(ctx, hipMemcpyAsync(h.data(), R->lens.p, (uint64_t)n_reads * 4, hipMemcpyDeviceToHost, ctx->stream));
 		HIP_TRY(ctx, hipStreamSynchronize(ctx->stream));
-		uint64_t tb = 0; for (uint32_t l : h) tb += l;
+		uint64_t tb = 0; for (uint32_t l : h) { tb += l; R->max_len = std::max(R->max_len, l); }
 		R->total_bases = tb;
 	}
 	HIP_TRY(ctx, hipStreamSynchronize(ctx->stream));
diff --git a/colord_amd/csrc/objects.hpp b/colord_amd/csrc/objects.hpp
--- a/colord_amd/csrc/objects.hpp
+++ b/colord_amd/csrc/objects.hpp
@@ -6,6 +6,7 @@
 	cl_ctx* ctx = nullptr;
 	uint32_t n_reads = 0;
 	uint64_t total_bases = 0, total_words = 0;
+	uint32_t max_len = 0;
 	DevBuf<uint64_t> packed;
 	DevBuf<uint32_t> inv;
 	DevBuf<uint64_t> word_off;
diff --git a/colord_amd/csrc/pairsort.hip b/colord_amd/csrc/pairsort.hip
--- /dev/null
+++ b/colord_amd/csrc/pairsort.hip
@@ -0,0 +1,148 @@
+#include "common.hpp"
+#include <cstdlib>
+
+namespace {
+constexpr uint32_t TIE_LANE = 8, TIE_LANE_MAX = 32;
+constexpr uint32_t TIE_BLOCK = 2048, TIE_NT = 256;
+
+__global__ __launch_bounds__(256) void k_tie_heads(uint64_t* keys, uint32_t n, uint32_t pr, uint32_t lane_max,
+                                                   uint32_t* __restrict__ list, uint32_t list_cap, uint32_t* __restrict__ cnt)
+{
+	const uint64_t i = (uint64_t)blockIdx.x * 256 + threadIdx.x;
+	bool run2 = false;
+	if (i < n)
+	{
+		const uint64_t h = keys[i] >> pr;
+		const bool head = i == 0 || (keys[i - 1] >> pr) != h;
+		if (head && i + 1 < n && (keys[i + 1] >> pr) == h)
+		{
+			run2 = true;
+			uint32_t len = 2;
+			while (len <= lane_max && i + len < n && (keys[i + len] >> pr) == h) ++len;
+			if (len <= lane_max)
+			{
+				uint64_t* k = keys + i;
+				for (uint32_t a = 1; a < len; ++a)
+				{
+					const uint64_t v = k[a];
+					uint32_t b = a;
+					for (; b > 0 && k[b - 1] > v; --b) k[b] = k[b - 1];
+					k[b] = v;
+				}
+			}
+			else
+			{
+				const uint32_t at = atomicAdd(cnt + 1, 1u);
+				if (at < list_cap) list[at] = (uint32_t)i;
+			}
+		}
+	}
+	const uint64_t b = __ballot(run2);
+	if ((threadIdx.x & 63) == 0 && b) atomicAdd(cnt, (uint32_t)__popcll(b));
+}
+
+__global__ __launch_bounds__(TIE_NT) void k_tie_blocks(uint64_t* keys, uint32_t n, uint32_t pr, uint32_t block_max,
+                                                       const uint32_t* __restrict__ list, uint32_t list_cap, uint32_t* __restrict__ cnt)
+{
+	__shared__ uint64_t sk[TIE_BLOCK];
+	__shared__ uint32_t s_len;
+	const uint32_t n_list = min(cnt[1], list_cap);
+	for (uint32_t r = blockIdx.x; r < n_list; r += gridDim.x)
+	{
+		const uint32_t s = list[r];
+		const uint64_t h = keys[s] >> pr;
+		if (threadIdx.x == 0) s_len = block_max + 1;
+		__syncthreads();
+		for (uint32_t j0 = 0; j0 <= block_max; j0 += TIE_NT)
+		{
+			const uint32_t j = j0 + threadIdx.x;
+			if (j <= block_max)
+			{
+				const uint64_t idx = (uint64_t)s + j;
+				uint64_t k = 0;
+				bool in = idx < n;
+				if (in) { k = keys[idx]; in = (k >> pr) == h; }
+				if (!in) atomicMin(&s_len, j);
+				else if (j < block_max) sk[j] = k;
+			}
+			__syncthreads();
+			const bool ended = s_len < j0 + TIE_NT;
+			__syncthreads();
+			if (ended) break;
+		}
+		const uint32_t len = s_len;
+		if (len > block_max)
+		{
+			if (threadIdx.x == 0) atomicAdd(cnt + 2, 1u);
+		}
+		else
+		{
+			uint32_t P = 2; while (P < len) P <<= 1;
+			for (uint32_t j = len + threadIdx.x; j < P; j += TIE_NT) sk[j] = ~0ull;
+			__syncthreads();
+			for (uint32_t k = 2; k <= P; k <<= 1)
+				for (uint32_t j = k >> 1; j > 0; j >>= 1)
+				{
+					for (uint32_t t = threadIdx.x; t < P / 2; t += TIE_NT)
+					{
+						const uint32_t lo = ((t & ~(j - 1)) << 1) | (t & (j - 1)), hi = lo | j;
+						const bool up = (lo & k) == 0;
+						const uint64_t a = sk[lo], b = sk[hi];
+						if ((a > b) == up) { sk[lo] = b; sk[hi] = a; }
+					}
+					__syncthreads();
+				}
+			for (uint32_t j = threadIdx.x; j < len; j += TIE_NT) keys[(uint64_t)s + j] = sk[j];
+		}
+		__syncthreads();
+	}
+}
+
+__global__ void k_tie_report(const uint32_t* __restrict__ cnt, uint64_t* __restrict__ slot)
+{
+	slot[0] = cnt[0]; slot[1] = cnt[1]; slot[2] = cnt[2];
+}
+
+uint32_t env_bound(const char* name, uint32_t dflt, uint32_t lo, uint32_t hi)
+{
+	const char* e = getenv(name);
+	return e ? (uint32_t)std::min<long>(hi, std::max<long>(lo, atol(e))) : dflt;
+}
+}
+
+cl_status dev_pair_sort(cl_ctx* ctx, uint64_t* d_keys, uint64_t n, uint32_t pr_bits, uint32_t hi_bits, PairSortStats* st)
+{
+	PairSortStats S; S.pairs = n; S.pr = pr_bits; S.hi = hi_bits;
+	auto done = [&](cl_status s) { if (s == CL_OK) { ctx->pair_sort.add(S); if (st) *st = S; } return s; };
+	if (pr_bits + hi_bits > 64) return cl_fail(ctx, CL_E_INVALID, "pair sort: " + std::to_string(pr_bits) + " + " + std::to_string(hi_bits) + " key bits are more than 64");
+	if (n >= (1ull << 32)) return cl_fail(ctx, CL_E_UNSUPPORTED, "pair sort: n must be < 2^32 per call");
+	const char* full = getenv("COLORD_HIP_PAIR_SORT_FULL");
+	if ((full && atoi(full) > 0) || pr_bits == 0 || hi_bits == 0)
+	{
+		S.full = 1;
+		return done(dev_sort_pairs(ctx, d_keys, nullptr, n, 0, pr_bits + hi_bits));
+	}
+	if (n < 2) return done(CL_OK);
+	const uint32_t lane_max = env_bound("COLORD_HIP_PAIR_TIE_LANE", TIE_LANE, 1, TIE_LANE_MAX);
+	const uint32_t block_max = env_bound("COLORD_HIP_PAIR_TIE_BLOCK", TIE_BLOCK, lane_max, TIE_BLOCK);
+	const uint32_t list_cap = (uint32_t)(n / (lane_max + 1)) + 1;
+	DevBuf<uint32_t> list, cnt; DEV_ALLOC(ctx, list, list_cap); DEV_ALLOC(ctx, cnt, 3);
+	uint64_t *hs = nullptr, *ds = nullptr;
+	HIP_TRY(ctx, cl_slot(ctx, 3, &hs, &ds));
+	const std::function<cl_status()> ties = [&]() -> cl_status {
+		HIP_TRY(ctx, hipMemsetAsync(cnt.p, 0, 12, cl_launch_stream(ctx)));
+		LAUNCHB(ctx, n * 8.0, k_tie_heads, grid_for(n, 256), 256, d_keys, (uint32_t)n, pr_bits, lane_max, list.p, list_cap, cnt.p);
+		LAUNCH(ctx, k_tie_blocks, std::min(list_cap, 1024u), TIE_NT, d_keys, (uint32_t)n, pr_bits, block_max, (const uint32_t*)list.p, list_cap, cnt.p);
+		LAUNCH(ctx, k_tie_report, 1, 1, (const uint32_t*)cnt.p, ds);
+		HIP_TRY(ctx, hipGetLastError());
+		return CL_OK;
+	};
+	CL_TRY(dev_sort_pairs_then(ctx, d_keys, n, pr_bits, pr_bits + hi_bits, ties));
+	S.runs = ((volatile uint64_t*)hs)[0]; S.block_runs = ((volatile uint64_t*)hs)[1];
+	if (((volatile uint64_t*)hs)[2])
+	{
+		S.fallbacks = 1;
+		return done(dev_sort_pairs(ctx, d_keys, nullptr, n, 0, pr_bits + hi_bits));
+	}
+	return done(CL_OK);
+}
diff --git a/colord_amd/csrc/sort.hip b/colord_amd/csrc/sort.hip
--- a/colord_amd/csrc/sort.hip
+++ b/colord_amd/csrc/sort.hip
@@ -1,4 +1,5 @@
 #include "common.hpp"
+#include <functional>
 #include <string>
 
 namespace {
@@ -152,11 +153,16 @@
 }
 
 template<typename K>
-cl_status sort_impl(cl_ctx* ctx, K* d_keys, uint32_t* d_vals, uint64_t n, uint32_t begin_bit, uint32_t end_bit, DevBuf<K>* swap_k = nullptr, DevBuf<uint32_t>* swap_v = nullptr)
+cl_status sort_impl(cl_ctx* ctx, K* d_keys, uint32_t* d_vals, uint64_t n, uint32_t begin_bit, uint32_t end_bit, DevBuf<K>* swap_k = nullptr, DevBuf<uint32_t>* swap_v = nullptr,
+                    const std::function<cl_status()>* after = nullptr)
 {
 	if (end_bit > 8 * sizeof(K)) return cl_fail(ctx, CL_E_INVALID, "radix sort: end_bit " + std::to_string(end_bit) + " is beyond the key's " + std::to_string(8 * sizeof(K)) + " bits");
-	if (n <= 1 || end_bit <= begin_bit) return CL_OK;
 	if (n >= (1ULL << 32)) return cl_fail(ctx, CL_E_UNSUPPORTED, "radix sort: n must be < 2^32 per call");
+	if (n <= 1 || end_bit <= begin_bit)
+	{
+		if (after) { CL_TRY((*after)()); HIP_TRY(ctx, hipStreamSynchronize(cl_launch_stream(ctx))); }
+		return CL_OK;
+	}
 	const uint32_t nb = grid_for(n, STILE);
 	const uint32_t bits = end_bit - begin_bit;
 	const uint32_t n_pass_real = (bits + 7) / 8 == (bits + 9) / 10 ? (bits + 7) / 8 : (bits + 9) / 10;
@@ -194,6 +200,7 @@
 		HIP_TRY(ctx, hipMemcpyAsync(d_keys, kin, n * sizeof(K), hipMemcpyDeviceToDevice, cl_launch_stream(ctx)));
 		if (d_vals) HIP_TRY(ctx, hipMemcpyAsync(d_vals, vin, n * 4, hipMemcpyDeviceToDevice, cl_launch_stream(ctx)));
 	}
+	if (after) CL_TRY((*after)());
 	HIP_TRY(ctx, hipStreamSynchronize(cl_launch_stream(ctx)));
 	return CL_OK;
 }
@@ -203,6 +210,10 @@
 {
 	return sort_impl<uint64_t>(ctx, d_keys, d_vals, n, begin_bit, end_bit);
 }
+cl_status dev_sort_pairs_then(cl_ctx* ctx, uint64_t* d_keys, uint64_t n, uint32_t begin_bit, uint32_t end_bit, const std::function<cl_status()>& after)
+{
+	return sort_impl<uint64_t>(ctx, d_keys, nullptr, n, begin_bit, end_bit, nullptr, nullptr, &after);
+}
 cl_status dev_sort_pairs_swap(cl_ctx* ctx, DevBuf<uint64_t>& keys, DevBuf<uint32_t>& vals, uint64_t n, uint32_t begin_bit, uint32_t end_bit)
 {
 	if (keys.n != n || vals.n != n) return sort_impl<uint64_t>(ctx, keys.p, vals.p, n, begin_bit, end_bit);
diff --git a/colord_amd/device.py b/colord_amd/device.py
--- a/colord_amd/device.py
+++ b/colord_amd/device.py
@@ -45,7 +45,7 @@
                   "cl_compressor_verified", "cl_ctx_set_verify_streams", "cl_ctx_verified_streams", "cl_compressor_verified_streams",
                   "cl_ctx_set_digest", "cl_ctx_digest", "cl_compressor_digest", "cl_digest_bases_host", "cl_digest_bytes_host", "cl_qual_decoder_set_digest", "cl_qual_decoder_digest",
                   "cl_ctx_set_digest_values", "cl_ctx_digest_values", "cl_compressor_digest_values", "cl_qual_values_host", "cl_digest_qual_values_host",
-                  "cl_qual_coder_domains", "cl_compressor_qual_domains", "cl_ctx_gap_paths",
+                  "cl_qual_coder_domains", "cl_compressor_qual_domains", "cl_ctx_gap_paths", "cl_ctx_pair_sort_stats",
                   "cl_report_clear", "cl_report_add", "cl_report_bases_host", "cl_report_quals_host", "cl_report_values_host", "cl_ctx_set_report", "cl_ctx_report", "cl_compressor_report")
 
     def __init__(self, lib, device):
@@ -117,6 +117,11 @@
         _check(None, self.lib.cl_ctx_gap_paths(self.h, out, 11))
         v = [int(x) for x in out]
         return {"classes": v[:8], "quad_to_wave": v[8], "giant_to_wave": v[9], "wave_redo_rounds": v[10]}
+
+    def pair_sort_stats(self) -> dict:
+        out = (C.c_uint64 * 8)()
+        _check(None, self.lib.cl_ctx_pair_sort_stats(self.h, out, 8))
+        return dict(zip(("calls", "pairs", "runs", "block_runs", "fallbacks", "full", "pr_bits", "hi_bits"), (int(x) for x in out)))
 
     def set_verify_streams(self, on: bool = True):
         self.lib.cl_ctx_set_verify_streams(self.h, int(bool(on)))
@@ -533,6 +538,12 @@
         _check(self, f(self.h, keys.data_ptr(), keys.numel(), shift, seg.data_ptr(), seg.numel(), C.byref(r)))
         return r.value
 
+    def pair_sort(self, keys: torch.Tensor, pr_bits: int, hi_bits: int) -> dict:
+        assert keys.dtype == torch.int64
+        st = (C.c_uint64 * 8)()
+        _check(self, self.lib.cl_pair_sort_u64(self.h, keys.data_ptr(), keys.numel(), pr_bits, hi_bits, st))
+        return dict(zip(("pairs", "runs", "block_runs", "fallback", "full", "pr_bits", "hi_bits", "calls"), (int(v) for v in st)))
+
 
 class _Obj:
     _free = None
diff --git a/include/colord_hip.h b/include/colord_hip.h
--- a/include/colord_hip.h
+++ b/include/colord_hip.h
@@ -36,6 +36,7 @@
 void cl_ctx_set_verify_streams(cl_ctx* ctx, int on);
 cl_status cl_ctx_verified_streams(const cl_ctx* ctx, uint64_t* parts, uint64_t* symbols, uint64_t* bytes);
 cl_status cl_ctx_gap_paths(const cl_ctx* ctx, uint64_t* out, uint32_t cap);
+cl_status cl_ctx_pair_sort_stats(const cl_ctx* ctx, uint64_t* out, uint32_t cap);
 typedef struct cl_digest { uint64_t reads, symbols, sum; } cl_digest;
 void cl_ctx_set_digest(cl_ctx* ctx, int on);
 cl_status cl_ctx_digest(const cl_ctx* ctx, cl_digest* dna, cl_digest* qual);
@@ -301,6 +302,7 @@
 cl_status cl_scan_u32_u64(cl_ctx* ctx, const uint32_t* d_in, uint64_t* d_out, uint64_t n, uint64_t* h_total);
 cl_status cl_run_starts_u32(cl_ctx* ctx, const uint32_t* d_keys, uint64_t n, uint32_t shift, uint32_t* d_seg, uint64_t seg_cap, uint64_t* h_n_runs);
 cl_status cl_run_starts_u64(cl_ctx* ctx, const uint64_t* d_keys, uint64_t n, uint32_t shift, uint32_t* d_seg, uint64_t seg_cap, uint64_t* h_n_runs);
+cl_status cl_pair_sort_u64(cl_ctx* ctx, uint64_t* d_keys, uint64_t n, uint32_t pr_bits, uint32_t hi_bits, uint64_t* h_stats);
 
 #ifdef __cplusplus
 }
```

Result: slower. 2.876 (-4.0%).
